# lajoiepy/cslam

Hardware: AMD Instinct MI355X
Metric: keyframes/sec (extract+match) on 100kx4096-D bank (higher is better)
Workload: dtype f32

## Files before the change

cslam_amd/_lib.py:

```python
import ctypes as C
import os
import subprocess

_HERE = os.path.dirname(os.path.abspath(__file__))
LIB_PATH = os.environ.get("CSLAM_HIP_LIB") or os.path.join(_HERE, "libcslam_hip.so")
CSRC_DIR = os.path.join(_HERE, "csrc")

F32, F64 = 0, 1
MODE_AUTO, MODE_SCAN, MODE_MFMA = 0, 1, 2


class CslamHipError(RuntimeError):
    pass


class CslamGraphError(CslamHipError):
    """CSLAM_E_GRAPH: the graph admits no Fiedler pair (not connected, singular junction Laplacian, TraceMIN breakdown) --
    the condition under which the reference's networkx call raises and acm.py:436-466 re-draws its start point.  Not a
    failure of the GPU path."""


class CslamUnsupportedError(CslamHipError):
    """CSLAM_E_UNSUPPORTED: an optional run-time dependency (RCCL, rocBLAS / rocSOLVER) was not found on this host."""


class CslamLimitError(CslamHipError):
    """CSLAM_E_LIMIT: valid input beyond a size limit of this entry point (cslam_fiedler: junctions of the dense factor)."""


_ERROR_CLASSES = {-5: CslamUnsupportedError, -6: CslamGraphError, -7: CslamLimitError}

_lib = None

_vp, _i, _i64, _f = C.c_void_p, C.c_int, C.c_int64, C.c_float
_SIGNATURES = {
    "cslam_last_error": (C.c_char_p, []),
    "cslam_version": (_i, []),
    "cslam_device_count": (_i, [C.POINTER(_i)]),
    "cslam_device_info": (_i, [_i, C.c_char_p, _i, C.POINTER(_i64), C.POINTER(_i)]),
    "cslam_bank_create": (_i, [_i, _i, _i64, C.POINTER(_vp)]),
    "cslam_bank_destroy": (_i, [_vp]),
    "cslam_bank_size": (_i, [_vp, C.POINTER(_i64), C.POINTER(_i)]),
    "cslam_bank_clear": (_i, [_vp]),
    "cslam_bank_add_host": (_i, [_vp, _vp, _i, _i64]),
    "cslam_bank_add_dev": (_i, [_vp, _vp, _i64, _i64, _vp]),
    "cslam_bank_read_host": (_i, [_vp, _i64, _i64, _vp]),
    "cslam_bank_device_ptr": (_i, [_vp, C.POINTER(_vp), C.POINTER(_i64)]),
    "cslam_bank_search_host": (_i, [_vp, _vp, _i, _i64, _i, _vp, _i, _vp, _vp, _vp]),
    "cslam_bank_search_dev": (_i, [_vp, _vp, _i, _i64, _i64, _i, _vp, _i, _vp, _vp, _vp, _vp]),
    "cslam_bank_search_multi_dev": (_i, [_vp, _i, _vp, _i, _i64, _i64, _vp, _vp, _i, _vp, _vp, _vp, _vp]),
    "cslam_bank_search_enqueue_dev": (_i, [_vp, _vp, _i, _i64, _i64, _i, _vp, _i, _vp, _vp, _vp, _vp]),
    "cslam_bank_search_finish": (_i, [_vp, C.POINTER(_i64)]),
    "cslam_bank_search_flag_copy_dev": (_i, [_vp, _vp, _vp]),
    "cslam_bank_search_multi_enqueue_dev": (_i, [_vp, _i, _vp, _i, _i64, _i64, _vp, _vp, _i, _vp, _vp, _vp, _vp]),
    "cslam_bank_search_multi_finish": (_i, [_vp, _i, C.POINTER(_i64)]),
    "cslam_bank_last_stats": (_i, [_vp, C.POINTER(_i64 * 4)]),
    "cslam_bank_last_stage": (_i, [_vp, C.POINTER(C.c_int32 * 4)]),
    "cslam_bank_last_kernel_ms": (_i, [_vp, C.POINTER(_f)]),
    "cslam_topk_merge_dev": (_i, [_vp, _vp, _vp, _vp, _i, _i64, _i, _vp, _vp, _vp, _vp]),
    "cslam_l2_normalize_dev": (_i, [_vp, _i64, _i, _i64, _f, _i, _vp]),
    "cslam_vlad_aggregate_dev": (_i, [_vp, _vp, _vp, _vp, _i, _i, _i, _i, _vp, _i64, _vp]),
    "cslam_vlad_aggregate_nhwc_dev": (_i, [_vp, _vp, _vp, _vp, _i, _i, _i, _i, _vp, _i64, _vp]),
    "cslam_gem_fc_head_dev": (_i, [_vp, _f, _f, _vp, _vp, _i, _i, _i, _i, _vp, _vp]),
    "cslam_gem_fc_head_nhwc_dev": (_i, [_vp, _f, _f, _vp, _vp, _i, _i, _i, _i, _vp, _vp]),
    "cslam_pca_project_dev": (_i, [_vp, _i64, _vp, _i64, _vp, _vp, _i, _i, _i, _vp, _vp]),
    "cslam_pca_project_pairs_dev": (_i, [_vp, _i64, C.c_float, _vp, C.c_float, _i, _vp, _vp, _i, _i, _i, _vp, _vp]),
    "cslam_preprocess_dev": (_i, [_vp, _i, _i, _i, _i, _i, C.POINTER(_f * 3), C.POINTER(_f * 3), _vp, _vp]),
    "cslam_preprocess_nhwc_dev": (_i, [_vp, _i, _i, _i, _i, _i, C.POINTER(_f * 3), C.POINTER(_f * 3), _vp, _vp]),
    "cslam_mac_grad_dev": (_i, [_vp, _vp, _vp, _vp, _i64, _vp, _vp]),
    "cslam_csr_spmm_dev": (_i, [_vp, _vp, _vp, _i64, _vp, _i, _vp, _vp]),
    "cslam_csr_spmm4_dev": (_i, [_vp, _vp, _vp, _i64, _vp, _vp, _vp]),
    "cslam_block4_gram_dev": (_i, [_vp, _vp, _i64, _vp, _vp, _vp]),
    "cslam_block4_affine_dev": (_i, [_vp, _i64, _vp, _vp, _vp, _vp]),
    "cslam_block4_residual_dev": (_i, [_vp, _vp, _i64, _vp, C.c_double, _vp, _vp, _vp]),
    "cslam_block4_gram_sync": (_i, [_vp, _vp, _i64, _vp, _vp, _vp, _vp]),
    "cslam_block4_affine_host": (_i, [_vp, _i64, _vp, _vp, _vp, _vp]),
    "cslam_block4_residual_sync": (_i, [_vp, _vp, _i64, _vp, C.c_double, _vp, _vp, _vp, _vp]),
    "cslam_chain_forward_dev": (_i, [_vp, _vp, _vp, _i64, _vp, _i, _vp, _vp, _vp, _vp, _vp, _vp, _vp, _vp, _vp, _vp, _vp]),
    "cslam_chain_backward_dev": (_i, [_vp, _vp, _vp, _vp, _vp, _vp, _vp, _vp, _vp, _vp, _i64, _vp, _vp]),
    "cslam_chol_solve4_dev": (_i, [_vp, _i64, _i64, _i, _vp, _vp, _i, _vp, _vp, _vp]),
    "cslam_fiedler": (_i, [_i64, _vp, _vp, _vp, _vp, C.c_uint32, C.c_double, _i, _vp, _vp, _vp, _vp]),
    "cslam_fiedler_start_block": (_i, [C.c_uint32, _i64, _vp]),
    "cslam_fiedler_release": (_i, []),
    "cslam_mac_fw_subset": (_i, [_i64, _i64, _vp, _vp, _vp, _i64, _vp, _vp, _vp, _vp, _i64, _i, C.c_double, C.c_double, _vp, _vp, _vp, _vp, _vp]),
    "cslam_pgo_plan": (_i, [_i64, _i64, _vp, _vp, _i64, _vp]),
    "cslam_pgo_linearize_dev": (_i, [_vp, _vp, _vp, _vp, _vp, _vp]),
    "cslam_pgo_system_host": (_i, [_vp, _vp, _vp, _vp, _vp, _vp]),
    "cslam_pgo_solve_dev": (_i, [C.c_double, _vp, _vp, _vp, _vp]),
    "cslam_pgo_retract_dev": (_i, [_vp, _vp, _i64, _vp, _vp]),
    "cslam_pgo_cost_dev": (_i, [_vp, _vp, _vp, _vp, _vp, _vp, _vp]),
    "cslam_pgo_weights_dev": (_i, [_vp, _i64, C.c_double, C.c_double, _vp, _vp, _vp]),
    "cslam_pgo_optimize": (_i, [_i64, _i64, _vp, _vp, _i64, _vp, _vp, _vp, _vp, _vp, _vp, _vp]),
    "cslam_pgo_trace": (_i, [_vp, _i64, _vp]),
    "cslam_pgo_release": (_i, []),
    "cslam_scbank_create": (_i, [_i, _i, _i, _i64, _vp]),
    "cslam_scbank_destroy": (_i, [_vp]),
    "cslam_scbank_size": (_i, [_vp, _vp, _vp, _vp]),
    "cslam_scbank_clear": (_i, [_vp]),
    "cslam_scbank_add_host": (_i, [_vp, _vp, _i64]),
    "cslam_scbank_add_dev": (_i, [_vp, _vp, _i64, _vp]),
    "cslam_scbank_read_host": (_i, [_vp, _i64, _i64, _vp, _vp]),
    "cslam_scbank_search_host": (_i, [_vp, _vp, _i64, _i, _vp, _vp, _vp, _vp, _vp, _vp, _vp]),
    "cslam_scbank_search_dev": (_i, [_vp, _vp, _i64, _i, _vp, _vp, _vp, _vp, _vp, _vp, _vp, _vp]),
    "cslam_bias_act_pool_dev": (_i, [_vp, _vp, _i, _i, _i, _i, _i, _i, _vp, _vp]),
    "cslam_conv3x3_c3_dev": (_i, [_vp, _vp, _vp, _i, _i, _i, _i, _i, _vp, _vp]),
    "cslam_wino_input_dev": (_i, [_vp, _i, _i, _i, _i, _vp, _vp]),
    "cslam_wino_output_dev": (_i, [_vp, _vp, _vp, _i, _i, _i, _i, _i, _i, _vp, _vp]),
    "cslam_wino4_input_dev": (_i, [_vp, _i, _i, _i, _i, _vp, _vp]),
    "cslam_wino4_output_dev": (_i, [_vp, _vp, _vp, _i, _i, _i, _i, _i, _i, _vp, _vp]),
    "cslam_absmax_dev": (_i, [_vp, _i64, _vp, _vp]),
    "cslam_wino4_input_h3_dev": (_i, [_vp, _i, _i, _i, _i, _vp, _vp, _vp]),
    "cslam_wino4_output_scaled_dev": (_i, [_vp, _vp, _vp, _i, _i, _i, _i, _i, _i, _vp, C.c_float, _vp, _vp, _vp]),
    "cslam_wino2_fused64_dev": (_i, [_vp, _vp, _vp, _i, _i, _i, _i, _i, _vp, _vp]),
    "cslam_wino2_fused_c64_dev": (_i, [_vp, _vp, _vp, _vp, _i, _i, _i, _i, _i, _i, _vp, _vp]),
    "cslam_wino4_fused_c64_dev": (_i, [_vp, _vp, _vp, _vp, _i, _i, _i, _i, _i, _i, _vp, _vp]),
    "cslam_scancontext_from_cloud_dev": (_i, [_vp, _vp, _i, _i, _i, C.c_double, _vp, _vp, _vp]),
    "cslam_icp_correspondences_dev": (_i, [_vp, _vp, _vp, _vp, _i, _vp, C.c_double, _vp, _vp, _vp]),
    "cslam_icp_register_dev": (_i, [_vp, _vp, _vp, _vp, _i, _vp, _vp, _vp, _i, C.c_double, C.c_double, _vp, _vp, _vp]),
    "cslam_icp_register_plane_dev": (_i, [_vp, _vp, _vp, _vp, _vp, _i, _vp, _vp, _vp, _i, C.c_double, C.c_double, _vp, _vp, _vp]),
    "cslam_voxel_downsample_dev": (_i, [_vp, _vp, _i, C.c_double, _vp, _vp, _vp, _vp, _vp, _vp]),
    "cslam_knn_radius_dev": (_i, [_vp, _vp, _i, C.c_double, _i, _vp, _vp, _vp, _vp, _vp]),
    "cslam_normals_dev": (_i, [_vp, _vp, _i, _vp, _vp, _vp, _i, C.c_double, _i, _vp, _vp, _vp, _vp]),
    "cslam_fpfh_dev": (_i, [_vp, _vp, _vp, _i, _vp, _vp, _vp, _i, _vp, _vp, _vp, _vp]),
    "cslam_feature_match_dev": (_i, [_vp, _vp, _vp, _vp, _i, _i, _vp, _vp, _vp, _vp, _vp, _vp, _vp]),
    "cslam_robust_graph_dev": (_i, [_vp, _vp, _vp, _vp, _i, C.c_double, _vp, _vp, _vp, _vp, _vp, _vp]),
    "cslam_robust_clique_dev": (_i, [_vp, _vp, _vp, _vp, _vp, _i, _i64, _vp, _vp, _vp, _vp, _vp, _vp, _vp]),
    "cslam_robust_rotation_dev": (_i, [_vp, _vp, _vp, _vp, _vp, _i, C.c_double, _vp, _vp, _vp, _vp, _vp]),
    "cslam_robust_translation_dev": (_i, [_vp, _vp, _vp, _vp, _vp, _vp, _i, C.c_double, _vp, _vp, _vp, _vp]),
    "cslam_robust_fit_dev": (_i, [_vp, _vp, _vp, _vp, _vp, _vp, _vp, _i, C.c_double, _i64, _vp, _vp, _vp, _vp, _vp, _vp]),
    "cslam_vis_match_dev": (_i, [_vp, _vp, _vp, _vp, _i, _i, C.c_double, _vp, _vp, _vp, _vp, _vp]),
    "cslam_vis_pnp_dev": (_i, [_vp, _vp, _vp, _vp, _vp, _vp, _vp, _vp, _i, _i, C.c_double, _i, _i, _i, C.c_uint64, _vp, _vp, _vp, _vp]),
    "cslam_vis_register_dev": (_i, [_vp, _vp, _vp, _vp, _vp, _vp, _vp, _i, _i, C.c_double, _i, C.c_double, _i, _i, _i, C.c_uint64,
                                    _vp, _vp, _vp, _vp, _vp, _vp, _vp, _vp]),
    "cslam_vis_hypotheses_dev": (_i, [_vp, _vp, _vp, _vp, _i, _i, C.c_double, C.c_uint64, _vp, _vp, _vp, _vp, _vp, _vp, _vp]),
    "cslam_wino4_fused_c64_h_dev": (_i, [_vp, _vp, _vp, _vp, _i, _i, _i, _i, _i, _i, _vp, C.c_float, _vp, _vp, _vp]),
    "cslam_conv3x3_direct_h_dev": (_i, [_vp, _vp, _vp, _i, _i, _i, _i, _i, _i, _i, _vp, _f, _vp, _vp, _vp]),
    "cslam_conv3x3_direct_r_dev": (_i, [_vp, _vp, _vp, _i, _i, _i, _i, _i, _i, _i, _vp, C.c_float, _vp, _vp, _vp]),
    "cslam_conv3x3_direct_r2_dev": (_i, [_vp, _vp, _vp, _i, _i, _i, _i, _i, _i, _i, _vp, C.c_float, _vp, _vp, _vp]),
    "cslam_conv_stem_direct_h_dev": (_i, [_vp, _vp, _vp, _vp, C.c_float, _vp, _vp, C.c_float, _i, _i, _i, _i, _vp, _vp, _vp, _vp]),
    "cslam_wino4_stem_c64_h_dev": (_i, [_vp, _vp, _vp, _vp, C.c_float, _vp, _vp, _i, _i, _i, _i, _vp, C.c_float, _vp, _vp, _vp]),
    "cslam_debug_wfh_prof_dev": (_i, [_vp]),
    "cslam_conv3x3_c3_amax_dev": (_i, [_vp, _vp, _vp, _i, _i, _i, _i, _i, _vp, _vp, _vp]),
    "cslam_wino4_input_h2_dev": (_i, [_vp, _i, _i, _i, _i, _vp, _vp, _vp]),
    "cslam_wino_gemm_h2_dev": (_i, [_vp, _vp, _i64, _i, _i, _vp, _vp]),
    "cslam_wino4_chain_h2_dev": (_i, [_vp, _vp, _i, _i, _i, _i, _vp, C.c_float, _vp, C.c_float, C.c_float, _vp, _vp, _vp, _vp]),
    "cslam_wino_zgemm_h2_dev": (_i, [_vp, _vp, _i64, _i, _i, _vp, _vp]),
    "cslam_wino4_output_z_dev": (_i, [_vp, _vp, _i, _i, _i, _i, _i, _i, _vp, C.c_float, _vp, _vp, _vp]),
    "cslam_conv_igemm_h2_dev": (_i, [_vp, _vp, _vp, _vp, _i, _i, _i, _i, _i, _i, _i, _i, _i, _i, _vp, C.c_float, _vp, _vp, _vp]),
    "cslam_conv_stem_pool_igemm_h2_dev": (_i, [_vp, _vp, _vp, _i, _i, _i, _i, _i, _i, _i, _i, _vp, C.c_float, _vp, _vp, _vp]),
    "cslam_conv_igemm_h2p_dev": (_i, [_vp, _i, _vp, _vp, _vp, _vp, _i, _vp, _i, _i, _i, _i, _i, _i, _i, _i, _i, _i, _vp, C.c_float,
                                      C.c_float, C.c_float, _vp, _i, _vp, _vp, _vp]),
    "cslam_conv3x3_direct_r_pairs_dev": (_i, [_vp, _vp, _vp, _i, _i, _i, _i, _i, _vp, C.c_float, C.c_float, C.c_float, _vp, _vp, _vp, _vp]),
    "cslam_conv3x3_direct_hp_dev": (_i, [_vp, _vp, _vp, _vp, _i, _i, _i, _i, _i, _i, _i, C.c_float, _vp, _vp, _vp]),
    "cslam_conv3x3_direct_p_dev": (_i, [_vp, _i, _vp, _vp, _vp, _vp, _i, _vp, _i, _i, _i, _i, _i, _i, _vp, C.c_float, C.c_float, C.c_float,
                                        _vp, _i, _vp, _vp, _vp]),
    "cslam_comm_unique_id": (_i, [_vp]),
    "cslam_comm_init": (_i, [_i, _i, _vp, _i, C.POINTER(_vp)]),
    "cslam_comm_destroy": (_i, [_vp]),
    "cslam_comm_info": (_i, [_vp, C.POINTER(_i), C.POINTER(_i)]),
    "cslam_allgather_queries_dev": (_i, [_vp, _vp, _i64, _i64, _vp, _vp]),
    "cslam_exchange_lists_dev": (_i, [_vp, _vp, _vp, _i64, _vp]),
    "cslam_peak_copy_dev": (_i, [_vp, _vp, _i64, _i, _vp]),
    "cslam_peak_mfma_dev": (_i, [_i, _i, _i, _i, _vp, C.POINTER(C.c_double), _vp]),
    "cslam_debug_last_candidates": (_i, [_vp, _i64, C.POINTER(_i), _vp, _vp, C.POINTER(C.c_double)]),
    "cslam_ring_schedule_describe": (_i, [_i, _i, _i, _i, C.POINTER(C.c_int32 * 6), _vp, _i64, _vp, _vp, _vp]),
    "cslam_trunk_timing": (_i, [_i]),
    "cslam_trunk_timing_read": (_i, [C.POINTER(C.c_double * 8)]),
    "cslam_voxel_profile": (_i, [_i]),
    "cslam_voxel_profile_read": (_i, [C.POINTER(C.c_double * 6), C.POINTER(C.c_int32 * 4)]),
}

EXPERIMENTAL_SYMBOLS = ("cslam_wino4_input_h3_dev", "cslam_wino2_fused64_dev", "cslam_wino2_fused_c64_dev",
                        "cslam_wino4_fused_c64_dev", "cslam_debug_wfh_prof_dev", "cslam_peak_copy_dev", "cslam_peak_mfma_dev",
                        "cslam_debug_last_candidates", "cslam_ring_schedule_describe", "cslam_trunk_timing", "cslam_trunk_timing_read",
                        "cslam_voxel_profile", "cslam_voxel_profile_read", "cslam_vis_hypotheses_dev")
EXPORTED_SYMBOLS = tuple(n for n in _SIGNATURES if n not in EXPERIMENTAL_SYMBOLS)


def build(verbose=False):
    r = subprocess.run(["make", "-C", CSRC_DIR, "-j", "4"], capture_output=True, text=True)
    if verbose or r.returncode != 0:
        print(r.stdout[-4000:])
        print(r.stderr[-4000:])
    if r.returncode != 0:
        raise CslamHipError("building libcslam_hip.so failed")
    return LIB_PATH


def load():
    global _lib
    if _lib is not None:
        return _lib
    try:
        import torch
    except ImportError:
        pass
    if not os.path.exists(LIB_PATH):
        raise CslamHipError(
            f"{LIB_PATH} not found: the HIP extension is not built "
            "(run `python __graft_entry__.py` or `make -C cslam_amd/csrc`); there is no CPU fallback")
    lib = C.CDLL(LIB_PATH)
    for name, (res, args) in _SIGNATURES.items():
        fn = getattr(lib, name)
        fn.restype = res
        fn.argtypes = args
    _lib = lib
    return lib


def check(rc):
    if rc != 0:
        msg = load().cslam_last_error()
        raise _ERROR_CLASSES.get(rc, CslamHipError)(f"libcslam_hip error {rc}: {msg.decode() if msg else ''}")


def require_gpu():
    lib = load()
    n = C.c_int(0)
    rc = lib.cslam_device_count(C.byref(n))
    if rc != 0 or n.value < 1:
        msg = lib.cslam_last_error()
        raise CslamHipError("no HIP device visible: cslam_amd needs an MI355X (gfx950); "
                            f"no CPU fallback exists ({msg.decode() if msg else ''})")
    return n.value
```

cslam_amd/csrc/conv_direct_r.hip:

```cpp
#include <stdlib.h>
#include <type_traits>
#include <hip/hip_fp16.h>
#include "common.h"
#include "pairs.h"

typedef float f32x4 __attribute__((ext_vector_type(4)));
typedef unsigned u32x4 __attribute__((ext_vector_type(4)));
typedef _Float16 f16x8 __attribute__((ext_vector_type(8)));
typedef float dr_f32x2 __attribute__((ext_vector_type(2)));

#define DR_PP 320
#define DR_SWZ(pc) (((pc) >> 1) & 3)
#define DR_RP (18 * DR_PP)
#define DR_PATCHB (10 * DR_RP)
#define DR_NPIX 180
#define DR_NEL 12
#define DR_SINKB 4096
#define DR_LDS (2 * DR_PATCHB + DR_SINKB)
#define DR_SINK_END (63 * 16 + 128 + 8)

struct ConvDirectRArgs {
    const float *x; const f16x8 *w2; const float *bias; float *y;
    int B, H, W, gxb, gyb, nblk;
    int relu;
    const unsigned *amax_in; float inv_sw; unsigned *amax_out;
    float wl1, bmax; unsigned *bound_out;
};

#ifdef CSLAM_ABLATIONS
__device__ unsigned long long *dr_prof = nullptr;
extern "C" __attribute__((visibility("default"))) int cslam_debug_dr_prof_dev(void *d_buf) {
    unsigned long long *q = (unsigned long long *)d_buf;
    return hipMemcpyToSymbol(HIP_SYMBOL(dr_prof), &q, sizeof(q)) == hipSuccess ? 0 : -2;
}
#define DR_PROF 1
#else
#define DR_PROF 0
#endif

template <bool POOL, bool RELU, int DBG = 0, bool OUTP = false>
__global__ __launch_bounds__(256, 1) void conv3x3_direct_r_kernel(ConvDirectRArgs p) {
    static_assert(!(POOL && OUTP), "the pair-format output is written un-pooled");
    static_assert(DR_SINK_END <= DR_SINKB, "a sink store leaves the sink");
    extern __shared__ __attribute__((aligned(16))) char dr_smem[];
    const int tid = threadIdx.x;
    const int lane = tid & 63;
    const int wave = __builtin_amdgcn_readfirstlane(tid >> 6);
    const int gq = lane >> 4, l15 = lane & 15;

    const float amax = fminf(fmaxf(__uint_as_float(*p.amax_in), 1e-30f), 1e30f);
    const float sx = scale_le_32752(__uint_as_float(*p.amax_in));
    const float inv = p.inv_sw / sx;
    float s_out = 1.0f, neg1 = -1.0f;
    asm volatile("" : "+v"(neg1));
    if (OUTP) {
        const float bound = (amax * p.wl1 + p.bmax) * 1.001f;
        s_out = scale_in_2p13_2p14(bound);
        if (blockIdx.x == 0 && threadIdx.x == 0) *p.bound_out = __float_as_uint(bound);
    }

    const bool by_xcd = (gridDim.x & 7) == 0;
    const int wg_xcd = by_xcd ? (int)blockIdx.x & 7 : 0, wg_j = by_xcd ? (int)blockIdx.x >> 3 : (int)blockIdx.x;
    const int wg_per = by_xcd ? (int)gridDim.x >> 3 : (int)gridDim.x;
    const int per_xcd = by_xcd ? (p.nblk + 7) >> 3 : p.nblk;
    const int blk_beg = wg_xcd * per_xcd;
    const int blk_cnt = min(per_xcd, p.nblk - blk_beg);
    const int n_mine = blk_cnt > wg_j ? (blk_cnt - wg_j + wg_per - 1) / wg_per : 0;
    if (n_mine <= 0) return;

    f16x8 wr[9][2][2][2];
#pragma unroll
    for (int tap = 0; tap < 9; ++tap)
#pragma unroll
        for (int ks = 0; ks < 2; ++ks)
#pragma unroll
            for (int mt = 0; mt < 2; ++mt)
#pragma unroll
                for (int hl = 0; hl < 2; ++hl) {
                    wr[tap][ks][mt][hl] = p.w2[((((wave * 9 + tap) * 2 + ks) * 2 + mt) * 2 + hl) * 64 + lane];
                    if (tap < 6) asm volatile("" : "+a"(wr[tap][ks][mt][hl]));
                }
    float4 bv[2];
#pragma unroll
    for (int mt = 0; mt < 2; ++mt)
        bv[mt] = p.bias ? *(const float4 *)(p.bias + 32 * wave + 16 * mt + 4 * gq) : make_float4(0.f, 0.f, 0.f, 0.f);

    struct Blk { int img, by, bx; };
    auto decode_blk = [&](int bi) {
        int blk = wg_j + bi * wg_per;
        blk = blk_beg + (blk < blk_cnt ? blk : blk_cnt - 1);
        const int per_img = p.gxb * p.gyb;
        Blk b;
        b.img = blk / per_img;
        const int rem = blk - b.img * per_img;
        b.by = rem / p.gxb; b.bx = rem - b.by * p.gxb;
        return b;
    };

    int st_dst[DR_NEL];
    unsigned st_pc = 0;
#pragma unroll
    for (int i = 0; i < DR_NEL; ++i) {
        const int e = i * 256 + tid, px = e >> 4, f4 = e & 15;
        const int pr = (px * 3641) >> 16, pc = px - 18 * pr;
        const bool valid = px < DR_NPIX;
        st_dst[i] = valid ? pr * DR_RP + pc * DR_PP + (((f4 >> 1) ^ DR_SWZ(pc)) << 4) + (f4 & 1) * 8 : -1;
        if (i < 6) st_pc |= (unsigned)(valid ? pc : 0) << (5 * i);
    }
    unsigned st_pc2 = 0;
#pragma unroll
    for (int i = 6; i < DR_NEL; ++i) {
        const int e = i * 256 + tid, px = e >> 4;
        const int pr = (px * 3641) >> 16, pc = px - 18 * pr;
        st_pc2 |= (unsigned)(px < DR_NPIX ? pc : 0) << (5 * (i - 6));
    }
    const int img_bytes = p.H * p.W * 256;
    u32x4 stg[DR_NEL];
    auto patch_load = [&](const Blk &b, int i) {
        const __amdgpu_buffer_rsrc_t rsX = buf_rsrc((const char *)p.x + (int64_t)b.img * img_bytes, img_bytes, RSRC_LIM16);
        const int blk_off = ((b.by * 8 - 1) * p.W + (b.bx * 16 - 1)) * 256;
        int t = tid;
        asm volatile("" : "+v"(t));
        const int e = i * 256 + t, px = e >> 4;
        const int pr = (px * 3641) >> 16, pc = px - 18 * pr;
        int off = ((pr * p.W + pc) * 64 + (e & 15) * 4) * 4 + blk_off;
        asm volatile("" : "+v"(off));
        stg[i] = __builtin_amdgcn_raw_buffer_load_b128(rsX, px < DR_NPIX ? off : 0x7fffffff, 0, 0);
    };
    auto patch_split = [&](const Blk &b, int i, char *patch) {
        const unsigned pc = __builtin_amdgcn_ubfe(i < 6 ? st_pc : st_pc2, 5 * (i < 6 ? i : i - 6), 5);
        const float s = (unsigned)(b.bx * 16 - 1) + pc < (unsigned)p.W ? sx : 0.0f;
        dr_f32x2 w01 = dr_f32x2{__uint_as_float(stg[i].x), __uint_as_float(stg[i].y)} * dr_f32x2{s, s};
        dr_f32x2 w23 = dr_f32x2{__uint_as_float(stg[i].z), __uint_as_float(stg[i].w)} * dr_f32x2{s, s};
        asm("" : "+v"(w01), "+v"(w23));
        const float w0 = w01[0], w1 = w01[1], w2 = w23[0], w3 = w23[1];
        const __half2 h01 = __floats2half2_rn(w0, w1), h23 = __floats2half2_rn(w2, w3);
        const float d0 = sub_half<0>(w0, h01), d1 = sub_half<1>(w1, h01), d2 = sub_half<0>(w2, h23), d3 = sub_half<1>(w3, h23);
        const __half2 l01 = __floats2half2_rn(d0, d1), l23 = __floats2half2_rn(d2, d3);
        char *d = st_dst[i] >= 0 ? patch + st_dst[i] : dr_smem + 2 * DR_PATCHB + (tid & 63) * 16;
        *(uint2 *)d = make_uint2(*(const unsigned *)&h01, *(const unsigned *)&h23);
        *(uint2 *)(d + 128) = make_uint2(*(const unsigned *)&l01, *(const unsigned *)&l23);
    };

    f32x4 acc[8][2];
    int fr_off[3];
#pragma unroll
    for (int dx = 0; dx < 3; ++dx) fr_off[dx] = (l15 + dx) * DR_PP + ((gq ^ DR_SWZ(l15 + dx)) << 4);
    f16x8 fh[3], fl[3];
    auto frag_read = [&](auto col_tag, auto r_tag, const char *patch) {
        constexpr int COL = decltype(col_tag)::value, R = decltype(r_tag)::value;
        constexpr int DX = COL >> 1, KS = COL & 1, SLOT = (R + COL) % 3;
        fh[SLOT] = *(const f16x8 *)(patch + fr_off[DX] + R * DR_RP + KS * 64);
        fl[SLOT] = *(const f16x8 *)(patch + fr_off[DX] + R * DR_RP + KS * 64 + 128);
    };
    float my_amax = 0.0f;
    const int Ho = POOL ? p.H >> 1 : p.H, Wo = POOL ? p.W >> 1 : p.W;
    Blk eb = {0, 0, 0};
    auto epi_rows = [&](int k) {
        const __amdgpu_buffer_rsrc_t rsY = buf_rsrc((const char *)(p.y + (int64_t)eb.img * Ho * Wo * 128), (int64_t)Ho * Wo * 512, RSRC_LIM16);
        const int ox = eb.bx * 16 + l15;
#pragma unroll
        for (int mt = 0; mt < 2; ++mt) {
            const int ch_off = (32 * wave + 16 * mt + 4 * gq) * 4;
            float4 v;
            bool store;
            int off;
            if (POOL) {
                const int py = eb.by * 4 + k;
                v.x = max_f32_xor1(max_f32(acc[2 * k][mt][0], acc[2 * k + 1][mt][0])); v.y = max_f32_xor1(max_f32(acc[2 * k][mt][1], acc[2 * k + 1][mt][1]));
                v.z = max_f32_xor1(max_f32(acc[2 * k][mt][2], acc[2 * k + 1][mt][2])); v.w = max_f32_xor1(max_f32(acc[2 * k][mt][3], acc[2 * k + 1][mt][3]));
                store = ((l15 & 1) == 0) & ((ox >> 1) < Wo) & (py < Ho);
                off = (py * Wo + (ox >> 1)) * 512 + ch_off;
            } else {
                const int oy = eb.by * 8 + k;
                v.x = acc[k][mt][0]; v.y = acc[k][mt][1]; v.z = acc[k][mt][2]; v.w = acc[k][mt][3];
                store = (ox < p.W) & (oy < p.H);
                off = (oy * p.W + ox) * 512 + ch_off;
            }
            v.x = v.x * inv + bv[mt].x; v.y = v.y * inv + bv[mt].y; v.z = v.z * inv + bv[mt].z; v.w = v.w * inv + bv[mt].w;
            if (RELU) { v.x = fmaxf(v.x, 0.0f); v.y = fmaxf(v.y, 0.0f); v.z = fmaxf(v.z, 0.0f); v.w = fmaxf(v.w, 0.0f); }
            float m = max_f32(max_f32(fabsf(v.x), fabsf(v.y)), max_f32(fabsf(v.z), fabsf(v.w)));
            asm volatile("" : "+v"(m), "+v"(off));
            my_amax = max_f32(my_amax, store ? m : 0.0f);
            if (OUTP) {
                const float u0 = v.x * s_out, u1 = v.y * s_out, u2 = v.z * s_out, u3 = v.w * s_out;
                const unsigned h01 = pack_half2(u0, u1), h23 = pack_half2(u2, u3);
                const unsigned l01 = pack_half2(fma_half<0>(h01, neg1, u0), fma_half<1>(h01, neg1, u1));
                const unsigned l23 = pack_half2(fma_half<0>(h23, neg1, u2), fma_half<1>(h23, neg1, u3));
                const int offp = store ? off - ch_off + wave * 128 + (16 * mt + 4 * gq) * 2 : 0x7fffffff;
                typedef unsigned dr_u32x2 __attribute__((ext_vector_type(2)));
                __builtin_amdgcn_raw_buffer_store_b64((dr_u32x2){h01, h23}, rsY, offp, 0, 0);
                __builtin_amdgcn_raw_buffer_store_b64((dr_u32x2){l01, l23}, rsY, offp, 64, 0);
            } else {
            u32x4 bits;
            bits.x = __float_as_uint(v.x); bits.y = __float_as_uint(v.y); bits.z = __float_as_uint(v.z); bits.w = __float_as_uint(v.w);
            if (!(DBG & 4)) __builtin_amdgcn_raw_buffer_store_b128(bits, rsY, store ? off : 0x7fffffff, 0, 0);
            else asm volatile("" :: "v"(bits));
            }
        }
    };

    auto rstep = [&](auto col_tag, auto r_tag, const char *patch, const Blk &nblk, char *npatch) {
        constexpr int COL = decltype(col_tag)::value, R = decltype(r_tag)::value;
        constexpr int DX = COL >> 1, KS = COL & 1, SLOT = (R + COL) % 3;
        if constexpr (R + 2 < 10) frag_read(col_tag, std::integral_constant<int, (R + 2) % 10>{}, patch);
        else if constexpr (COL < 5) frag_read(std::integral_constant<int, (COL + 1) % 6>{}, std::integral_constant<int, (R + 2) % 10>{}, patch);
        if constexpr (COL == 0 && R >= 1 && R <= 6 && !(DBG & 1)) { patch_load(nblk, 2 * (R - 1)); patch_load(nblk, 2 * (R - 1) + 1); }
#pragma unroll
        for (int prod = 0; prod < 3; ++prod)
#pragma unroll
            for (int dy = 0; dy < 3; ++dy)
#pragma unroll
                for (int mt = 0; mt < 2; ++mt) {
                    const int r = R - dy;
                    if (r < 0 || r > 7) continue;
                    const f16x8 a = prod == 2 ? wr[3 * dy + DX][KS][mt][1] : wr[3 * dy + DX][KS][mt][0];
                    const f16x8 b = prod == 1 ? fl[SLOT] : fh[SLOT];
                    acc[r][mt] = __builtin_amdgcn_mfma_f32_16x16x32_f16(a, b, (COL == 0 && prod == 0 && dy == 0) ? (f32x4)(0.0f) : acc[r][mt], 0, 0, 0);
                }
        if constexpr (COL >= 3 && (R == 1 || R == 3 || R == 5 || R == 7) && !(DBG & 1)) patch_split(nblk, 4 * (COL - 3) + (R - 1) / 2, npatch);
        if constexpr (COL == 5 && !POOL && R >= 3) epi_rows(R - 3);
        if constexpr (COL == 5 && POOL && (R == 4 || R == 6 || R == 8)) epi_rows((R - 4) / 2);
        __builtin_amdgcn_sched_group_barrier(0x100, 2, 0);
        __builtin_amdgcn_sched_group_barrier(0x020, 2, 0);
        constexpr int NM = 6 * ((R < 2 ? R + 1 : 3) - (R > 7 ? R - 7 : 0));
#pragma unroll
        for (int m = 0; m < NM; ++m) {
            __builtin_amdgcn_sched_group_barrier(0x008, 1, 0);
            __builtin_amdgcn_sched_group_barrier(0x002, COL == 5 ? 4 : 2, 0);
        }
        __builtin_amdgcn_sched_group_barrier(0x200, 1, 0);
        __builtin_amdgcn_sched_barrier(0);
    };
    auto column = [&](auto col_tag, const char *patch, const Blk &nblk, char *npatch) {
        rstep(col_tag, std::integral_constant<int, 0>{}, patch, nblk, npatch); rstep(col_tag, std::integral_constant<int, 1>{}, patch, nblk, npatch);
        rstep(col_tag, std::integral_constant<int, 2>{}, patch, nblk, npatch); rstep(col_tag, std::integral_constant<int, 3>{}, patch, nblk, npatch);
        rstep(col_tag, std::integral_constant<int, 4>{}, patch, nblk, npatch); rstep(col_tag, std::integral_constant<int, 5>{}, patch, nblk, npatch);
        rstep(col_tag, std::integral_constant<int, 6>{}, patch, nblk, npatch); rstep(col_tag, std::integral_constant<int, 7>{}, patch, nblk, npatch);
        rstep(col_tag, std::integral_constant<int, 8>{}, patch, nblk, npatch); rstep(col_tag, std::integral_constant<int, 9>{}, patch, nblk, npatch);
    };
#define DR_C(T) std::integral_constant<int, T>{}

    [[maybe_unused]] unsigned long long t_main = 0, t_epi = 0, t_bar = 0, t1 = 0, t2 = 0, t3 = 0;
    Blk cb = decode_blk(0);
#pragma unroll
    for (int i = 0; i < DR_NEL; ++i) patch_load(cb, i);
#pragma unroll
    for (int i = 0; i < DR_NEL; ++i) patch_split(cb, i, dr_smem);
    __syncthreads();
    for (int bi = 0; bi < n_mine; ++bi) {
        const int cur = bi & 1;
        const char *const patch = dr_smem + cur * DR_PATCHB;
        char *const npatch = dr_smem + (cur ^ 1) * DR_PATCHB;
        const Blk nb = decode_blk(bi + 1);
        eb = cb;
        if (DR_PROF) t1 = __builtin_amdgcn_s_memtime();
        frag_read(DR_C(0), DR_C(0), patch);
        frag_read(DR_C(0), DR_C(1), patch);
        column(DR_C(0), patch, nb, npatch); column(DR_C(1), patch, nb, npatch); column(DR_C(2), patch, nb, npatch);
        column(DR_C(3), patch, nb, npatch); column(DR_C(4), patch, nb, npatch); column(DR_C(5), patch, nb, npatch);
        if (DR_PROF) { t2 = __builtin_amdgcn_s_memtime(); t_main += t2 - t1; }
        epi_rows(POOL ? 3 : 7);
        if (DR_PROF) { t3 = __builtin_amdgcn_s_memtime(); t_epi += t3 - t2; }
        __syncthreads();
        if (DR_PROF) t_bar += __builtin_amdgcn_s_memtime() - t3;
        cb = nb;
    }
#ifdef CSLAM_ABLATIONS
    if (dr_prof && blockIdx.x == 0 && tid == 0) { dr_prof[0] = t_main; dr_prof[1] = t_epi; dr_prof[2] = t_bar; dr_prof[3] = (unsigned long long)n_mine; }
#endif

    if (p.amax_out) {
        unsigned *s_amax = (unsigned *)dr_smem;
        if (tid == 0) *s_amax = 0u;
        __syncthreads();
#pragma unroll
        for (int o = 32; o > 0; o >>= 1) my_amax = fmaxf(my_amax, __shfl_xor(my_amax, o, 64));
        if (lane == 0) atomicMax(s_amax, __float_as_uint(my_amax));
        __syncthreads();
        if (tid == 0 && *s_amax > *(volatile unsigned *)p.amax_out) atomicMax(p.amax_out, *s_amax);
    }
}

typedef float f32x2 __attribute__((ext_vector_type(2)));
#define DR2_SINKB 1280
#define DR2_BUF (DR_PATCHB + DR2_SINKB)
#define DR2_LDS (2 * DR2_BUF)
struct ConvDirectR2Args {
    const float *x; const f16x8 *w2; const float *bias; float *y;
    int B, H, W, gxb, gyb, nblk;
    const unsigned *amax_in; float inv_sw; unsigned *amax_out;
};
template <bool POOL, bool RELU, int DBG = 0>
__global__ __launch_bounds__(256, 1) void conv3x3_direct_r2_kernel(ConvDirectR2Args p) {
    extern __shared__ __attribute__((aligned(16))) char dr_smem[];
    const int tid = threadIdx.x;
    const int lane = tid & 63;
    const int wave = __builtin_amdgcn_readfirstlane(tid >> 6);
    const int gq = lane >> 4, l15 = lane & 15;

    const float sx = scale_le_32752(__uint_as_float(*p.amax_in));
    const float inv = p.inv_sw / sx;

    const bool by_xcd = (gridDim.x & 15) == 0;
    const int wg_xcd = by_xcd ? (int)blockIdx.x & 7 : 0, wg_raw = by_xcd ? (int)blockIdx.x >> 3 : (int)blockIdx.x;
    const int half = wg_raw & 1, wg_j = wg_raw >> 1;
    const int wg_per = (by_xcd ? (int)gridDim.x >> 3 : (int)gridDim.x) >> 1;
    const int per_xcd = by_xcd ? (p.nblk + 7) >> 3 : p.nblk;
    const int blk_beg = wg_xcd * per_xcd;
    const int blk_cnt = min(per_xcd, p.nblk - blk_beg);
    const int n_mine = blk_cnt > wg_j ? (blk_cnt - wg_j + wg_per - 1) / wg_per : 0;
    if (n_mine <= 0) return;

    f16x8 wr[9][2][2][2];
#pragma unroll
    for (int tap = 0; tap < 9; ++tap)
#pragma unroll
        for (int ks = 0; ks < 2; ++ks)
#pragma unroll
            for (int sl = 0; sl < 2; ++sl)
#pragma unroll
                for (int hl = 0; hl < 2; ++hl) {
                    wr[tap][ks][sl][hl] = p.w2[((((((half * 4 + wave) * 9 + tap) * 2 + ks) * 2 + sl) * 2 + hl) * 64) + lane];
                    if (tap < 7) asm volatile("" : "+a"(wr[tap][ks][sl][hl]));
                }
    const float4 bv = p.bias ? *(const float4 *)(p.bias + 64 * half + 16 * wave + 4 * gq) : make_float4(0.f, 0.f, 0.f, 0.f);

    struct Blk { int img, by, bx; };
    auto decode_blk = [&](int bi) {
        int blk = wg_j + bi * wg_per;
        blk = blk_beg + (blk < blk_cnt ? blk : blk_cnt - 1);
        const int per_img = p.gxb * p.gyb;
        Blk b;
        b.img = blk / per_img;
        const int rem = blk - b.img * per_img;
        b.by = rem / p.gxb; b.bx = rem - b.by * p.gxb;
        return b;
    };

    static_assert(DR_SINK_END <= DR2_SINKB && DR2_BUF % 256 == 0, "a sink store leaves its sink, or the second buffer moves in the banks");
    int st_dst[DR_NEL], st_src[DR_NEL];
    unsigned st_pc = 0, st_pc2 = 0;
#pragma unroll
    for (int i = 0; i < DR_NEL; ++i) {
        const int e = i * 256 + tid, px = e >> 4, f4 = e & 15;
        const int pr = (px * 3641) >> 16, pc = px - 18 * pr;
        const bool valid = px < DR_NPIX;
        st_dst[i] = valid ? pr * DR_RP + pc * DR_PP + (((f4 >> 1) ^ DR_SWZ(pc)) << 4) + (f4 & 1) * 8 : DR_PATCHB + (tid & 63) * 16;
        st_src[i] = valid ? ((pr * p.W + pc) * 128 + f4 * 4) * 4 : -1;
        if (i < 6) st_pc |= (unsigned)(valid ? pc : 0) << (5 * i);
        else st_pc2 |= (unsigned)(valid ? pc : 0) << (5 * (i - 6));
    }
    const int img_bytes = p.H * p.W * 512;
    u32x4 stg[DR_NEL];
    auto patch_load = [&](const Blk &b, int slab, int i) {
        const __amdgpu_buffer_rsrc_t rsX = buf_rsrc((const char *)p.x + (int64_t)b.img * img_bytes, img_bytes, RSRC_LIM16);
        const int blk_off = ((b.by * 8 - 1) * p.W + (b.bx * 16 - 1)) * 512 + slab * 256;
        int off = st_src[i] + blk_off;
        asm volatile("" : "+v"(off));
        stg[i] = __builtin_amdgcn_raw_buffer_load_b128(rsX, st_src[i] >= 0 ? off : 0x7fffffff, 0, 0);
    };
    auto patch_split = [&](const Blk &b, int i, char *patch) {
        const unsigned pc = __builtin_amdgcn_ubfe(i < 6 ? st_pc : st_pc2, 5 * (i < 6 ? i : i - 6), 5);
        const float s = (unsigned)(b.bx * 16 - 1) + pc < (unsigned)p.W ? sx : 0.0f;
        f32x2 w01 = f32x2{__uint_as_float(stg[i].x), __uint_as_float(stg[i].y)} * f32x2{s, s};
        f32x2 w23 = f32x2{__uint_as_float(stg[i].z), __uint_as_float(stg[i].w)} * f32x2{s, s};
        asm("" : "+v"(w01), "+v"(w23));
        const __half2 h01 = __floats2half2_rn(w01[0], w01[1]), h23 = __floats2half2_rn(w23[0], w23[1]);
        const float d0 = sub_half<0>(w01[0], h01), d1 = sub_half<1>(w01[1], h01), d2 = sub_half<0>(w23[0], h23), d3 = sub_half<1>(w23[1], h23);
        const __half2 l01 = __floats2half2_rn(d0, d1), l23 = __floats2half2_rn(d2, d3);
        char *d = patch + st_dst[i];
        *(uint2 *)d = make_uint2(*(const unsigned *)&h01, *(const unsigned *)&h23);
        *(uint2 *)(d + 128) = make_uint2(*(const unsigned *)&l01, *(const unsigned *)&l23);
    };

    f32x4 acc[8];
    int fr_off[3];
#pragma unroll
    for (int dx = 0; dx < 3; ++dx) fr_off[dx] = (l15 + dx) * DR_PP + ((gq ^ DR_SWZ(l15 + dx)) << 4);
    f16x8 fh[3], fl[3];
    auto frag_read = [&](auto col_tag, auto r_tag, const char *patch) {
        constexpr int COL = decltype(col_tag)::value, R = decltype(r_tag)::value;
        constexpr int DX = COL >> 1, KS = COL & 1, SLOT = (R + COL) % 3;
        fh[SLOT] = *(const f16x8 *)(patch + fr_off[DX] + R * DR_RP + KS * 64);
        fl[SLOT] = *(const f16x8 *)(patch + fr_off[DX] + R * DR_RP + KS * 64 + 128);
    };
    float my_amax = 0.0f;
    const int Ho = POOL ? p.H >> 1 : p.H, Wo = POOL ? p.W >> 1 : p.W;
    Blk eb = {0, 0, 0};
    auto epi_rows = [&](int k) {
        const __amdgpu_buffer_rsrc_t rsY = buf_rsrc((const char *)(p.y + (int64_t)eb.img * Ho * Wo * 128), (int64_t)Ho * Wo * 512, RSRC_LIM16);
        const int ox = eb.bx * 16 + l15;
        const int ch_off = (64 * half + 16 * wave + 4 * gq) * 4;
        float4 v;
        bool store;
        int off;
        if (POOL) {
            const int py = eb.by * 4 + k;
            v.x = max_f32_xor1(max_f32(acc[2 * k][0], acc[2 * k + 1][0])); v.y = max_f32_xor1(max_f32(acc[2 * k][1], acc[2 * k + 1][1]));
            v.z = max_f32_xor1(max_f32(acc[2 * k][2], acc[2 * k + 1][2])); v.w = max_f32_xor1(max_f32(acc[2 * k][3], acc[2 * k + 1][3]));
            store = ((l15 & 1) == 0) & ((ox >> 1) < Wo) & (py < Ho);
            off = (py * Wo + (ox >> 1)) * 512 + ch_off;
        } else {
            const int oy = eb.by * 8 + k;
            v.x = acc[k][0]; v.y = acc[k][1]; v.z = acc[k][2]; v.w = acc[k][3];
            store = (ox < p.W) & (oy < p.H);
            off = (oy * p.W + ox) * 512 + ch_off;
        }
        v.x = v.x * inv + bv.x; v.y = v.y * inv + bv.y; v.z = v.z * inv + bv.z; v.w = v.w * inv + bv.w;
        if (RELU) { v.x = fmaxf(v.x, 0.0f); v.y = fmaxf(v.y, 0.0f); v.z = fmaxf(v.z, 0.0f); v.w = fmaxf(v.w, 0.0f); }
        float m = max_f32(max_f32(fabsf(v.x), fabsf(v.y)), max_f32(fabsf(v.z), fabsf(v.w)));
        asm volatile("" : "+v"(m), "+v"(off));
        my_amax = max_f32(my_amax, store ? m : 0.0f);
        u32x4 bits;
        bits.x = __float_as_uint(v.x); bits.y = __float_as_uint(v.y); bits.z = __float_as_uint(v.z); bits.w = __float_as_uint(v.w);
        if (!(DBG & 4)) __builtin_amdgcn_raw_buffer_store_b128(bits, rsY, store ? off : 0x7fffffff, 0, 0);
        else asm volatile("" :: "v"(bits));
    };

    auto rstep = [&](auto col_tag, auto r_tag, auto slab_tag, const char *patch, const Blk &nblk, int nslab, char *npatch) {
        constexpr int COL = decltype(col_tag)::value, R = decltype(r_tag)::value, SL = decltype(slab_tag)::value;
        constexpr int DX = COL >> 1, KS = COL & 1, SLOT = (R + COL) % 3;
        if constexpr (R + 2 < 10) frag_read(col_tag, std::integral_constant<int, (R + 2) % 10>{}, patch);
        else if constexpr (COL < 5) frag_read(std::integral_constant<int, (COL + 1) % 6>{}, std::integral_constant<int, (R + 2) % 10>{}, patch);
        if constexpr (COL == 0 && R >= 1 && R <= 6 && !(DBG & 1) && !(DBG & 8)) { patch_load(nblk, nslab, 2 * (R - 1)); patch_load(nblk, nslab, 2 * (R - 1) + 1); }
#pragma unroll
        for (int prod = 0; prod < 3; ++prod)
#pragma unroll
            for (int dy = 0; dy < 3; ++dy) {
                const int r = R - dy;
                if (r < 0 || r > 7) continue;
                const f16x8 a = prod == 2 ? wr[3 * dy + DX][KS][SL][1] : wr[3 * dy + DX][KS][SL][0];
                const f16x8 b = prod == 1 ? fl[SLOT] : fh[SLOT];
                acc[r] = __builtin_amdgcn_mfma_f32_16x16x32_f16(a, b, (SL == 0 && COL == 0 && prod == 0 && dy == 0) ? (f32x4)(0.0f) : acc[r], 0, 0, 0);
            }
        if constexpr (COL >= 3 && (R == 1 || R == 3 || R == 5 || R == 7) && !(DBG & 1) && !(DBG & 16)) patch_split(nblk, 4 * (COL - 3) + (R - 1) / 2, npatch);
        if constexpr (SL == 1 && COL == 5 && !POOL && R >= 3) epi_rows(R - 3);
        if constexpr (SL == 1 && COL == 5 && POOL && (R == 4 || R == 6 || R == 8)) epi_rows((R - 4) / 2);
        __builtin_amdgcn_sched_group_barrier(0x100, 2, 0);
        __builtin_amdgcn_sched_group_barrier(0x020, 2, 0);
        constexpr int NM = 3 * ((R < 2 ? R + 1 : 3) - (R > 7 ? R - 7 : 0));
#pragma unroll
        for (int m = 0; m < NM; ++m) {
            __builtin_amdgcn_sched_group_barrier(0x008, 1, 0);
            __builtin_amdgcn_sched_group_barrier(0x002, (SL == 1 && COL == 5) ? 8 : 4, 0);
        }
        __builtin_amdgcn_sched_group_barrier(0x200, 1, 0);
        __builtin_amdgcn_sched_barrier(0);
    };
    auto column = [&](auto col_tag, auto slab_tag, const char *patch, const Blk &nblk, int nslab, char *npatch) {
        rstep(col_tag, std::integral_constant<int, 0>{}, slab_tag, patch, nblk, nslab, npatch); rstep(col_tag, std::integral_constant<int, 1>{}, slab_tag, patch, nblk, nslab, npatch);
        rstep(col_tag, std::integral_constant<int, 2>{}, slab_tag, patch, nblk, nslab, npatch); rstep(col_tag, std::integral_constant<int, 3>{}, slab_tag, patch, nblk, nslab, npatch);
        rstep(col_tag, std::integral_constant<int, 4>{}, slab_tag, patch, nblk, nslab, npatch); rstep(col_tag, std::integral_constant<int, 5>{}, slab_tag, patch, nblk, nslab, npatch);
        rstep(col_tag, std::integral_constant<int, 6>{}, slab_tag, patch, nblk, nslab, npatch); rstep(col_tag, std::integral_constant<int, 7>{}, slab_tag, patch, nblk, nslab, npatch);
        rstep(col_tag, std::integral_constant<int, 8>{}, slab_tag, patch, nblk, nslab, npatch); rstep(col_tag, std::integral_constant<int, 9>{}, slab_tag, patch, nblk, nslab, npatch);
    };
    auto pass = [&](auto slab_tag, const char *patch, const Blk &nblk, int nslab, char *npatch) {
        frag_read(DR_C(0), DR_C(0), patch);
        frag_read(DR_C(0), DR_C(1), patch);
        column(DR_C(0), slab_tag, patch, nblk, nslab, npatch); column(DR_C(1), slab_tag, patch, nblk, nslab, npatch);
        column(DR_C(2), slab_tag, patch, nblk, nslab, npatch); column(DR_C(3), slab_tag, patch, nblk, nslab, npatch);
        column(DR_C(4), slab_tag, patch, nblk, nslab, npatch); column(DR_C(5), slab_tag, patch, nblk, nslab, npatch);
    };

    Blk cb = decode_blk(0);
#pragma unroll
    for (int i = 0; i < DR_NEL; ++i) patch_load(cb, 0, i);
#pragma unroll
    for (int i = 0; i < DR_NEL; ++i) patch_split(cb, i, dr_smem);
    __syncthreads();
    char *const buf0 = dr_smem, *const buf1 = dr_smem + DR2_BUF;
    for (int bi = 0; bi < n_mine; ++bi) {
        const Blk nb = decode_blk(bi + 1);
        eb = cb;
        pass(DR_C(0), buf0, cb, 1, buf1);
        __syncthreads();
        pass(DR_C(1), buf1, nb, 0, buf0);
        epi_rows(POOL ? 3 : 7);
        __syncthreads();
        cb = nb;
    }
    if (p.amax_out) {
        unsigned *s_amax = (unsigned *)dr_smem;
        if (tid == 0) *s_amax = 0u;
        __syncthreads();
#pragma unroll
        for (int o = 32; o > 0; o >>= 1) my_amax = fmaxf(my_amax, __shfl_xor(my_amax, o, 64));
        if (lane == 0) atomicMax(s_amax, __float_as_uint(my_amax));
        __syncthreads();
        if (tid == 0 && *s_amax > *(volatile unsigned *)p.amax_out) atomicMax(p.amax_out, *s_amax);
    }
}

CSLAM_API int cslam_conv3x3_direct_r2_dev(const float *d_x, const void *d_w2r2, const float *d_bias, int B, int H, int W, int Cin,
                                          int Cout, int relu, int pool, const unsigned *d_amax, float inv_sw,
                                          unsigned *d_amax_out, float *d_y, void *stream) {
    PTR_DEVICE(d_x);
    ARG_CHECK(d_x && d_w2r2 && d_y && d_amax, "NULL argument");
    ARG_CHECK(B >= 1 && H >= 1 && W >= 1, "empty map");
    ARG_CHECK(Cin == 128 && Cout == 128, "Cin and Cout must be 128");
    ARG_CHECK(!pool || ((H % 2) == 0 && (W % 2) == 0), "pooling needs even H and W");
    ARG_CHECK(inv_sw > 0.0f, "inv_sw must be positive");
    ARG_CHECK((int64_t)H * W * 512 < 0x7ffffff0ll, "one image's maps must stay below 2 GiB (32-bit buffer offsets)");
    ConvDirectR2Args a;
    a.x = d_x; a.w2 = (const f16x8 *)d_w2r2; a.bias = d_bias; a.y = d_y;
    a.B = B; a.H = H; a.W = W;
    a.gxb = (int)ceil_div64(W, 16); a.gyb = (int)ceil_div64(H, 8);
    const int64_t nblk = (int64_t)B * a.gxb * a.gyb;
    ARG_CHECK(nblk < (1ll << 30), "too many blocks for one launch");
    a.nblk = (int)nblk;
    a.amax_in = d_amax; a.inv_sw = inv_sw; a.amax_out = d_amax_out;
    const int n_cu = cslam_cu_count();
    ARG_CHECK(n_cu >= 2, "no HIP device");
    int grid = n_cu % 16 == 0 ? n_cu : (n_cu & ~1);
    if (2 * nblk < grid) grid = (int)(2 * nblk);
    hipStream_t st = (hipStream_t)stream;
#define DR2_LAUNCH(P, R) do { \
        static DeviceOnce once; int once_dev; \
        if (once.todo(&once_dev)) { \
            HIP_TRY(hipFuncSetAttribute((const void *)conv3x3_direct_r2_kernel<P, R>, hipFuncAttributeMaxDynamicSharedMemorySize, DR2_LDS)); \
            once.done(once_dev); } \
        hipLaunchKernelGGL((conv3x3_direct_r2_kernel<P, R>), dim3(grid), dim3(256), DR2_LDS, st, a); } while (0)
#ifdef CSLAM_ABLATIONS
    if (const char *e = getenv("CSLAM_DR_DBG")) {
        const int d = atoi(e);
#define DR2_LAUNCH_D(D) do { HIP_TRY(hipFuncSetAttribute((const void *)conv3x3_direct_r2_kernel<true, true, D>, hipFuncAttributeMaxDynamicSharedMemorySize, DR2_LDS)); \
        hipLaunchKernelGGL((conv3x3_direct_r2_kernel<true, true, D>), dim3(grid), dim3(256), DR2_LDS, st, a); HIP_TRY(hipGetLastError()); return CSLAM_OK; } while (0)
        if (d == 1) DR2_LAUNCH_D(1);
        if (d == 4) DR2_LAUNCH_D(4);
        if (d == 5) DR2_LAUNCH_D(5);
        if (d == 8) DR2_LAUNCH_D(8);
        if (d == 16) DR2_LAUNCH_D(16);
#undef DR2_LAUNCH_D
    }
#endif
    if (pool && relu) DR2_LAUNCH(true, true);
    else if (pool) DR2_LAUNCH(true, false);
    else if (relu) DR2_LAUNCH(false, true);
    else DR2_LAUNCH(false, false);
#undef DR2_LAUNCH
    HIP_TRY(hipGetLastError());
    return CSLAM_OK;
}

static int conv_direct_r_launch(const float *d_x, const void *d_w2r, const float *d_bias, int B, int H, int W, int Cin,
                                int Cout, int relu, int pool, const unsigned *d_amax, float inv_sw,
                                unsigned *d_amax_out, float *d_y, void *stream, int out_pairs, float wl1, float bmax, unsigned *d_bound_out) {
    PTR_DEVICE(d_x);
    ARG_CHECK(!out_pairs || (!pool && relu && d_bound_out && wl1 >= 0.0f && bmax >= 0.0f), "pair-format output: ReLU, no pooling, wl1, bmax and the bound slot");
    ARG_CHECK(d_x && d_w2r && d_y && d_amax, "NULL argument");
    ARG_CHECK(B >= 1 && H >= 1 && W >= 1, "empty map");
    ARG_CHECK(Cin == 64 && Cout == 128, "Cin must be 64 and Cout 128");
    ARG_CHECK(!pool || ((H % 2) == 0 && (W % 2) == 0), "pooling needs even H and W");
    ARG_CHECK(inv_sw > 0.0f, "inv_sw must be positive");
    ARG_CHECK((int64_t)H * W * 512 < 0x7ffffff0ll, "one image's maps must stay below 2 GiB (32-bit buffer offsets)");
    ConvDirectRArgs a;
    a.x = d_x; a.w2 = (const f16x8 *)d_w2r; a.bias = d_bias; a.y = d_y;
    a.B = B; a.H = H; a.W = W;
    a.gxb = (int)ceil_div64(W, 16); a.gyb = (int)ceil_div64(H, 8);
    const int64_t nblk = (int64_t)B * a.gxb * a.gyb;
    ARG_CHECK(nblk < (1ll << 30), "too many blocks for one launch");
    a.nblk = (int)nblk;
    a.relu = relu; a.amax_in = d_amax; a.inv_sw = inv_sw; a.amax_out = d_amax_out;
    a.wl1 = wl1; a.bmax = bmax; a.bound_out = d_bound_out;
    const int n_cu = cslam_cu_count();
    ARG_CHECK(n_cu > 0, "no HIP device");
    const int grid = (int)(nblk < n_cu ? nblk : n_cu);
    hipStream_t st = (hipStream_t)stream;
    if (out_pairs) {
        static DeviceOnce once_p; int once_dev_p;
        if (once_p.todo(&once_dev_p)) {
            HIP_TRY(hipFuncSetAttribute((const void *)conv3x3_direct_r_kernel<false, true, 0, true>, hipFuncAttributeMaxDynamicSharedMemorySize, DR_LDS));
            once_p.done(once_dev_p); }
        hipLaunchKernelGGL((conv3x3_direct_r_kernel<false, true, 0, true>), dim3(grid), dim3(256), DR_LDS, st, a);
        HIP_TRY(hipGetLastError());
        return CSLAM_OK;
    }
#define DR_LAUNCH(P, R) do { \
        static DeviceOnce once; int once_dev; \
        if (once.todo(&once_dev)) { \
            HIP_TRY(hipFuncSetAttribute((const void *)conv3x3_direct_r_kernel<P, R>, hipFuncAttributeMaxDynamicSharedMemorySize, DR_LDS)); \
            once.done(once_dev); } \
        hipLaunchKernelGGL((conv3x3_direct_r_kernel<P, R>), dim3(grid), dim3(256), DR_LDS, st, a); } while (0)
#ifdef CSLAM_ABLATIONS
    if (const char *e = getenv("CSLAM_DR_DBG")) {
        const int d = atoi(e);
#define DR_LAUNCH_D(D) do { HIP_TRY(hipFuncSetAttribute((const void *)conv3x3_direct_r_kernel<false, true, D>, hipFuncAttributeMaxDynamicSharedMemorySize, DR_LDS)); \
        hipLaunchKernelGGL((conv3x3_direct_r_kernel<false, true, D>), dim3(grid), dim3(256), DR_LDS, st, a); HIP_TRY(hipGetLastError()); return CSLAM_OK; } while (0)
        if (d == 1) DR_LAUNCH_D(1);
        if (d == 4) DR_LAUNCH_D(4);
        if (d == 5) DR_LAUNCH_D(5);
#undef DR_LAUNCH_D
    }
#endif
    if (pool && relu) DR_LAUNCH(true, true);
    else if (pool) DR_LAUNCH(true, false);
    else if (relu) DR_LAUNCH(false, true);
    else DR_LAUNCH(false, false);
#undef DR_LAUNCH
    HIP_TRY(hipGetLastError());
    return CSLAM_OK;
}
CSLAM_API int cslam_conv3x3_direct_r_dev(const float *d_x, const void *d_w2r, const float *d_bias, int B, int H, int W, int Cin,
                                         int Cout, int relu, int pool, const unsigned *d_amax, float inv_sw,
                                         unsigned *d_amax_out, float *d_y, void *stream) {
    return conv_direct_r_launch(d_x, d_w2r, d_bias, B, H, W, Cin, Cout, relu, pool, d_amax, inv_sw, d_amax_out, d_y, stream, 0, 0.0f, 0.0f, nullptr);
}
CSLAM_API int cslam_conv3x3_direct_r_pairs_dev(const float *d_x, const void *d_w2r, const float *d_bias, int B, int H, int W, int Cin,
                                               int Cout, const unsigned *d_amax, float inv_sw, float wl1, float bmax,
                                               unsigned *d_amax_out, unsigned *d_bound_out, void *d_y, void *stream) {
    return conv_direct_r_launch(d_x, d_w2r, d_bias, B, H, W, Cin, Cout, 1, 0, d_amax, inv_sw, d_amax_out, (float *)d_y, stream, 1, wl1, bmax, d_bound_out);
}
```

cslam_amd/csrc/conv_stem_direct_h.hip:

```cpp
#include <stdlib.h>
#include <type_traits>
#include <hip/hip_fp16.h>
#include "common.h"
#include "pairs.h"

typedef float f32x4 __attribute__((ext_vector_type(4)));
typedef unsigned u32x4 __attribute__((ext_vector_type(4)));
typedef _Float16 f16x8 __attribute__((ext_vector_type(8)));

#define SD_PP 320
#define SD_SWZ(pc) (((pc) >> 1) & 3)
#define SD_RP (18 * SD_PP)
#define SD_PATCHB (10 * SD_RP)
#define SD_IW 20
#define SD_IMG (12 * SD_IW * 3)
#define SD_T9 (20 * 17)
#define SD_IMGB (SD_IMG + SD_T9)
#define SD_NPIX 180
#define SD_LDS (2 * SD_PATCHB + 2 * SD_IMGB * 4)

struct StemDirectArgs {
    const float *x0; const unsigned *w1; const float *b1; const float *sumw; float inv_sw1;
    const f16x8 *w2; const float *bias; float inv_sw2;
    int B, H, W, gxb, gyb, nblk;
    const unsigned *amax_in; unsigned *amax_out; float *y;
};

#ifdef CSLAM_ABLATIONS
__device__ unsigned long long *sd_prof = nullptr;
extern "C" __attribute__((visibility("default"))) int cslam_debug_sd_prof_dev(void *d_buf) {
    unsigned long long *q = (unsigned long long *)d_buf;
    return hipMemcpyToSymbol(HIP_SYMBOL(sd_prof), &q, sizeof(q)) == hipSuccess ? 0 : -2;
}
#define SD_PROF 1
#else
#define SD_PROF 0
#endif

template <bool POOL, int DBG = 0>
__global__ __launch_bounds__(256, 1) void conv_stem_direct_h_kernel(StemDirectArgs p) {
    extern __shared__ __attribute__((aligned(16))) char sd_smem[];
    const int tid = threadIdx.x;
    const int lane = tid & 63;
    const int wave = __builtin_amdgcn_readfirstlane(tid >> 6);
    const int gq = lane >> 4, l15 = lane & 15;
    unsigned *const s_img_all = (unsigned *)(sd_smem + 2 * SD_PATCHB);

    const float a0 = fminf(fmaxf(__uint_as_float(*p.amax_in), 1e-30f), 1e30f);
    int e_;
    (void)frexpf(16384.0f / a0, &e_);
    const float s1 = ldexpf(1.0f, e_ - 1);
    const float inv1 = p.inv_sw1 / s1;
    float bound = 0.0f;
    for (int c = 0; c < 64; ++c) bound = fmaxf(bound, fabsf(p.b1 ? p.b1[c] : 0.0f) + a0 * p.sumw[c]);
    bound = fminf(fmaxf(bound, 1e-30f), 1e30f);
    (void)frexpf(32752.0f / bound, &e_);
    const float sx = ldexpf(1.0f, e_ - 1);
    const float inv2 = p.inv_sw2 / sx;

    const bool by_xcd = (gridDim.x & 7) == 0;
    const int wg_xcd = by_xcd ? (int)blockIdx.x & 7 : 0, wg_j = by_xcd ? (int)blockIdx.x >> 3 : (int)blockIdx.x;
    const int wg_per = by_xcd ? (int)gridDim.x >> 3 : (int)gridDim.x;
    const int per_xcd = by_xcd ? (p.nblk + 7) >> 3 : p.nblk;
    const int blk_beg = wg_xcd * per_xcd;
    const int blk_cnt = min(per_xcd, p.nblk - blk_beg);
    const int n_mine = blk_cnt > wg_j ? (blk_cnt - wg_j + wg_per - 1) / wg_per : 0;
    if (n_mine <= 0) return;

    f16x8 wr[9][2][2];
#pragma unroll
    for (int tap = 0; tap < 9; ++tap)
#pragma unroll
        for (int ks = 0; ks < 2; ++ks)
#pragma unroll
            for (int hl = 0; hl < 2; ++hl) {
                wr[tap][ks][hl] = p.w2[(((wave * 9 + tap) * 2 + ks) * 2 + hl) * 64 + lane];
                asm volatile("" : "+a"(wr[tap][ks][hl]));
            }
    const u32x4 w1h = ((const u32x4 *)p.w1)[(wave * 2 + 0) * 64 + lane], w1l = ((const u32x4 *)p.w1)[(wave * 2 + 1) * 64 + lane];
    const f16x8 W1h = __builtin_bit_cast(f16x8, w1h), W1l = __builtin_bit_cast(f16x8, w1l);
    const float k1 = inv1 * sx;
    float b1s[4];
#pragma unroll
    for (int r = 0; r < 4; ++r) b1s[r] = (p.b1 ? p.b1[16 * wave + 4 * gq + r] : 0.0f) * sx;
    float4 bv2;
    bv2 = p.bias ? *(const float4 *)(p.bias + 16 * wave + 4 * gq) : make_float4(0.f, 0.f, 0.f, 0.f);

    int e_dst[3], e_rc[3];
#pragma unroll
    for (int j = 0; j < 3; ++j) {
        const int e = j * 256 + tid;
        const int ci = (e >= 240) + (e >= 480);
        const int rem = e - 240 * ci;
        const int r = (rem * 3277) >> 16, c = rem - 20 * r;
        e_dst[j] = e < SD_IMG ? (r * SD_IW + c) * 3 + ci : -1;
        e_rc[j] = (ci << 16) | (r << 8) | c;
    }
    struct Blk { int img, by, bx; };
    auto decode_blk = [&](int bi) {
        int blk = wg_j + bi * wg_per;
        blk = blk_beg + (blk < blk_cnt ? blk : blk_cnt - 1);
        const int per_img = p.gxb * p.gyb;
        Blk b;
        b.img = blk / per_img;
        const int rem = blk - b.img * per_img;
        b.by = rem / p.gxb; b.bx = rem - b.by * p.gxb;
        return b;
    };
    float raw[3];
    auto img_load = [&](const Blk &b) {
#pragma unroll
        for (int j = 0; j < 3; ++j) {
            const int ci = e_rc[j] >> 16, r = (e_rc[j] >> 8) & 255, c = e_rc[j] & 255;
            const int gy = b.by * 8 - 2 + r, gx = b.bx * 16 - 2 + c;
            const bool in = (e_dst[j] >= 0) & (gy >= 0) & (gy < p.H) & (gx >= 0) & (gx < p.W);
            raw[j] = in ? p.x0[((int64_t)(b.img * 3 + ci) * p.H + gy) * p.W + gx] : 0.0f;
        }
    };
    auto img_store = [&](unsigned *s_img) {
#pragma unroll
        for (int j = 0; j < 3; ++j)
            if (e_dst[j] >= 0) {
                const unsigned v = pack_pair(raw[j] * s1);
                s_img[e_dst[j]] = v;
                if ((e_rc[j] >> 16) == 2) s_img[SD_IMG + (e_rc[j] & 255) * 17 + ((e_rc[j] >> 8) & 255)] = v;
            }
    };

    int c1_src[12], c1_dst[12];
#pragma unroll
    for (int t = 0; t < 12; ++t) {
        int pp = 16 * t + l15;
        pp = pp < SD_NPIX ? pp : SD_NPIX - 1;
        const int pr = (pp * 3641) >> 16, pc = pp - 18 * pr;
        c1_src[t] = (gq < 3 ? ((pr + gq) * SD_IW + pc) * 3 : SD_IMG + (pc + 2) * 17 + pr) * 4;
        c1_dst[t] = pr * SD_RP + pc * SD_PP + (((2 * wave + (gq >> 1)) ^ SD_SWZ(pc)) << 4) + (gq & 1) * 8;
    }
    for (int i = tid; i < 2 * 20 * 5; i += 256)
        s_img_all[(i / 100) * SD_IMGB + SD_IMG + ((i % 100) / 5) * 17 + 12 + (i % 5)] = 0u;
    unsigned pk[2][8];
    auto conv1_read = [&](int g, const unsigned *s_img) {
#pragma unroll
        for (int i = 0; i < 2; ++i) {
            const unsigned *ib = (const unsigned *)((const char *)s_img + c1_src[2 * g + i]);
#pragma unroll
            for (int j = 0; j < 8; ++j) pk[i][j] = ib[j];
        }
    };
    f32x4 c1[2];
    float c1v[2][4];
    auto conv1_piece = [&](int g, int piece, const Blk &b, char *patch) {
        const int i = piece & 1;
        if (piece < 2) {
            u32x4 ah, al;
#pragma unroll
            for (int d = 0; d < 4; ++d) {
                ah[d] = __builtin_amdgcn_perm(pk[i][2 * d + 1], pk[i][2 * d], 0x05040100u);
                al[d] = __builtin_amdgcn_perm(pk[i][2 * d + 1], pk[i][2 * d], 0x07060302u);
            }
            const f16x8 Ph = __builtin_bit_cast(f16x8, ah), Pl = __builtin_bit_cast(f16x8, al);
            c1[i] = __builtin_amdgcn_mfma_f32_16x16x32_f16(W1l, Ph, (f32x4)(0.0f), 0, 0, 0);
            c1[i] = __builtin_amdgcn_mfma_f32_16x16x32_f16(W1h, Pl, c1[i], 0, 0, 0);
            c1[i] = __builtin_amdgcn_mfma_f32_16x16x32_f16(W1h, Ph, c1[i], 0, 0, 0);
            asm volatile("" : "+v"(c1[i]));
            return;
        }
        if (piece < 4) {
#pragma unroll
            for (int r = 0; r < 4; ++r) c1v[i][r] = fmaxf(c1[i][r] * k1 + b1s[r], 0.0f);
            return;
        }
        const __half2 h01 = __floats2half2_rn(c1v[i][0], c1v[i][1]), h23 = __floats2half2_rn(c1v[i][2], c1v[i][3]);
        const float d0 = sub_half<0>(c1v[i][0], h01), d1 = sub_half<1>(c1v[i][1], h01);
        const float d2 = sub_half<0>(c1v[i][2], h23), d3 = sub_half<1>(c1v[i][3], h23);
        const __half2 l01 = __floats2half2_rn(d0, d1), l23 = __floats2half2_rn(d2, d3);
        if ((DBG & 16) == 0 && (2 * g + i < 11 || l15 < 4)) {
            char *d = patch + c1_dst[2 * g + i];
            *(uint2 *)d = make_uint2(*(const unsigned *)&h01, *(const unsigned *)&h23);
            *(uint2 *)(d + 128) = make_uint2(*(const unsigned *)&l01, *(const unsigned *)&l23);
        }
    };
    auto border_fixup = [&](const Blk &b, char *patch) {
        const int gy0 = b.by * 8 - 1, gx0 = b.bx * 16 - 1;
        if ((gy0 >= 0) & (gy0 + 10 <= p.H) & (gx0 >= 0) & (gx0 + 18 <= p.W)) return;
#pragma unroll
        for (int k = 0; k < 3; ++k) {
            const int pp = lane + 64 * k;
            const int pr = (pp * 3641) >> 16, pc = pp - 18 * pr;
            const int gy = gy0 + pr, gx = gx0 + pc;
            if (pp < SD_NPIX && !((gy >= 0) & (gy < p.H) & (gx >= 0) & (gx < p.W))) {
                char *d = patch + pr * SD_RP + pc * SD_PP;
                const int c0 = ((2 * wave) ^ SD_SWZ(pc)) << 4, c1_ = ((2 * wave + 1) ^ SD_SWZ(pc)) << 4;
                *(uint4 *)(d + c0) = make_uint4(0u, 0u, 0u, 0u); *(uint4 *)(d + c1_) = make_uint4(0u, 0u, 0u, 0u);
                *(uint4 *)(d + 128 + c0) = make_uint4(0u, 0u, 0u, 0u); *(uint4 *)(d + 128 + c1_) = make_uint4(0u, 0u, 0u, 0u);
            }
        }
    };

    float my_amax = 0.0f;
    const int Ho = POOL ? p.H >> 1 : p.H, Wo = POOL ? p.W >> 1 : p.W;
    f32x4 eacc[8];
    Blk ecb = {0, 0, 0};
    bool e_ok = false;
    auto epi_piece = [&](int k) {
        const __amdgpu_buffer_rsrc_t rsY = buf_rsrc((const char *)(p.y + (int64_t)ecb.img * Ho * Wo * 64), (int64_t)Ho * Wo * 256, RSRC_LIM16);
        const int ox = ecb.bx * 16 + l15;
        const int ch_off = (16 * wave + 4 * gq) * 4;
        if (POOL) {
            const int py = ecb.by * 4 + k;
            float4 v;
            v.x = max_f32_xor1(max_f32(eacc[2 * k][0], eacc[2 * k + 1][0])); v.y = max_f32_xor1(max_f32(eacc[2 * k][1], eacc[2 * k + 1][1]));
            v.z = max_f32_xor1(max_f32(eacc[2 * k][2], eacc[2 * k + 1][2])); v.w = max_f32_xor1(max_f32(eacc[2 * k][3], eacc[2 * k + 1][3]));
            v.x = fmaxf(v.x * inv2 + bv2.x, 0.0f); v.y = fmaxf(v.y * inv2 + bv2.y, 0.0f);
            v.z = fmaxf(v.z * inv2 + bv2.z, 0.0f); v.w = fmaxf(v.w * inv2 + bv2.w, 0.0f);
            const bool store = e_ok & ((l15 & 1) == 0) & ((ox >> 1) < Wo) & (py < Ho);
            float m = max_f32(max_f32(v.x, v.y), max_f32(v.z, v.w));
            int off = (py * Wo + (ox >> 1)) * 256 + ch_off;
            asm volatile("" : "+v"(m), "+v"(off));
            my_amax = max_f32(my_amax, store ? m : 0.0f);
            u32x4 bits;
            bits.x = __float_as_uint(v.x); bits.y = __float_as_uint(v.y); bits.z = __float_as_uint(v.z); bits.w = __float_as_uint(v.w);
            if (!(DBG & 4)) __builtin_amdgcn_raw_buffer_store_b128(bits, rsY, store ? off : 0x7fffffff, 0, 0);
        } else {
#pragma unroll
            for (int r = 2 * k; r < 2 * k + 2; ++r) {
                const int oy = ecb.by * 8 + r;
                float4 v;
                v.x = fmaxf(eacc[r][0] * inv2 + bv2.x, 0.0f); v.y = fmaxf(eacc[r][1] * inv2 + bv2.y, 0.0f);
                v.z = fmaxf(eacc[r][2] * inv2 + bv2.z, 0.0f); v.w = fmaxf(eacc[r][3] * inv2 + bv2.w, 0.0f);
                const bool store = e_ok & (ox < p.W) & (oy < p.H);
                float m = max_f32(max_f32(v.x, v.y), max_f32(v.z, v.w));
                int off = (oy * p.W + ox) * 256 + ch_off;
                asm volatile("" : "+v"(m), "+v"(off));
                my_amax = max_f32(my_amax, store ? m : 0.0f);
                u32x4 bits;
                bits.x = __float_as_uint(v.x); bits.y = __float_as_uint(v.y); bits.z = __float_as_uint(v.z); bits.w = __float_as_uint(v.w);
                __builtin_amdgcn_raw_buffer_store_b128(bits, rsY, store ? off : 0x7fffffff, 0, 0);
            }
        }
    };

    f32x4 acc[8];
    int fr_off[3];
#pragma unroll
    for (int dx = 0; dx < 3; ++dx) fr_off[dx] = (l15 + dx) * SD_PP + ((gq ^ SD_SWZ(l15 + dx)) << 4);
    f16x8 fh[3], fl[3];
    auto frag_read = [&](auto col_tag, auto r_tag, const char *patch) {
        constexpr int COL = decltype(col_tag)::value, R = decltype(r_tag)::value;
        constexpr int DX = COL >> 1, KS = COL & 1, SLOT = (R + COL) % 3;
        fh[SLOT] = *(const f16x8 *)(patch + fr_off[DX] + R * SD_RP + KS * 64);
        fl[SLOT] = *(const f16x8 *)(patch + fr_off[DX] + R * SD_RP + KS * 64 + 128);
    };
    auto rstep = [&](auto col_tag, auto r_tag, const char *patch, const unsigned *s_img, const Blk &nblk, char *npatch) {
        constexpr int COL = decltype(col_tag)::value, R = decltype(r_tag)::value;
        constexpr int DX = COL >> 1, KS = COL & 1, SLOT = (R + COL) % 3;
        if constexpr (DBG & 2) { }
        else if constexpr (R + 2 < 10) frag_read(col_tag, std::integral_constant<int, (R + 2) % 10>{}, patch);
        else if constexpr (COL < 5) frag_read(std::integral_constant<int, (COL + 1) % 6>{}, std::integral_constant<int, (R + 2) % 10>{}, patch);
        if constexpr (R == 0 && !(DBG & 1) && !(DBG & 8)) conv1_read(COL, s_img);
#pragma unroll
        for (int prod = 0; prod < 3; ++prod)
#pragma unroll
            for (int dy = 0; dy < 3; ++dy) {
                const int r = R - dy;
                if (r < 0 || r > 7) continue;
                const f16x8 a = prod == 2 ? wr[3 * dy + DX][KS][1] : wr[3 * dy + DX][KS][0];
                const f16x8 b = prod == 1 ? fl[SLOT] : fh[SLOT];
                acc[r] = __builtin_amdgcn_mfma_f32_16x16x32_f16(a, b, (COL == 0 && prod == 0 && dy == 0) ? (f32x4)(0.0f) : acc[r], 0, 0, 0);
            }
        if constexpr (R >= 2 && R <= 7 && !(DBG & 1)) conv1_piece(COL, R - 2, nblk, npatch);
        if constexpr (COL < 2 && (R == 1 || R == 8)) epi_piece(2 * COL + (R == 8 ? 1 : 0));
        __builtin_amdgcn_sched_group_barrier(0x100, R == 0 ? 18 : 2, 0);
        constexpr int NM = 3 * ((R < 2 ? R + 1 : 3) - (R > 7 ? R - 7 : 0)) + ((R == 2 || R == 3) ? 3 : 0);
#pragma unroll
        for (int m = 0; m < NM; ++m) {
            __builtin_amdgcn_sched_group_barrier(0x008, 1, 0);
            __builtin_amdgcn_sched_group_barrier(0x002, (COL < 2 && (R == 1 || R == 8)) ? 6 : 3, 0);
        }
        __builtin_amdgcn_sched_group_barrier(0x200, 2, 0);
        __builtin_amdgcn_sched_barrier(0);
    };
    auto edge = [&](auto col_tag, const char *patch, const unsigned *s_img) {
        constexpr int COL = decltype(col_tag)::value;
        constexpr int DX = COL >> 1, KS = COL & 1, SLOT = (9 + COL) % 3;
        constexpr int DX2 = (COL + 1) >> 1, KS2 = (COL + 1) & 1, SLOT2 = (COL + 1) % 3;
        if constexpr (!(DBG & 2)) frag_read(std::integral_constant<int, COL + 1>{}, std::integral_constant<int, 1>{}, patch);
        if constexpr (!(DBG & 1) && !(DBG & 8)) conv1_read(COL + 1, s_img);
#pragma unroll
        for (int prod = 0; prod < 3; ++prod) {
            acc[7] = __builtin_amdgcn_mfma_f32_16x16x32_f16(prod == 2 ? wr[6 + DX][KS][1] : wr[6 + DX][KS][0], prod == 1 ? fl[SLOT] : fh[SLOT], acc[7], 0, 0, 0);
            acc[0] = __builtin_amdgcn_mfma_f32_16x16x32_f16(prod == 2 ? wr[DX2][KS2][1] : wr[DX2][KS2][0], prod == 1 ? fl[SLOT2] : fh[SLOT2], acc[0], 0, 0, 0);
        }
        if constexpr (!(DBG & 2)) frag_read(std::integral_constant<int, COL + 1>{}, std::integral_constant<int, 2>{}, patch);
        __builtin_amdgcn_sched_group_barrier(0x100, 10, 0);
#pragma unroll
        for (int m = 0; m < 6; ++m) {
            __builtin_amdgcn_sched_group_barrier(0x008, 1, 0);
            __builtin_amdgcn_sched_group_barrier(0x002, 3, 0);
        }
        __builtin_amdgcn_sched_barrier(0);
    };
    auto column = [&](auto col_tag, const char *patch, const unsigned *s_img, const Blk &nblk, char *npatch) {
        constexpr int COL_ = decltype(col_tag)::value;
        if constexpr (COL_ == 0) rstep(col_tag, std::integral_constant<int, 0>{}, patch, s_img, nblk, npatch);
        rstep(col_tag, std::integral_constant<int, 1>{}, patch, s_img, nblk, npatch);
        rstep(col_tag, std::integral_constant<int, 2>{}, patch, s_img, nblk, npatch); rstep(col_tag, std::integral_constant<int, 3>{}, patch, s_img, nblk, npatch);
        rstep(col_tag, std::integral_constant<int, 4>{}, patch, s_img, nblk, npatch); rstep(col_tag, std::integral_constant<int, 5>{}, patch, s_img, nblk, npatch);
        rstep(col_tag, std::integral_constant<int, 6>{}, patch, s_img, nblk, npatch); rstep(col_tag, std::integral_constant<int, 7>{}, patch, s_img, nblk, npatch);
        rstep(col_tag, std::integral_constant<int, 8>{}, patch, s_img, nblk, npatch);
        if constexpr (COL_ == 5) rstep(col_tag, std::integral_constant<int, 9>{}, patch, s_img, nblk, npatch);
        else edge(col_tag, patch, s_img);
    };
#define SD_C(T) std::integral_constant<int, T>{}

    [[maybe_unused]] unsigned long long t_main = 0, t_epi = 0, t_bar = 0, t1 = 0, t2 = 0, t3 = 0;
    Blk cb = decode_blk(0);
    img_load(cb);
    img_store(s_img_all);
    Blk nb = decode_blk(1);
    img_load(nb);
    __syncthreads();
#pragma unroll
    for (int g = 0; g < 6; ++g) {
        conv1_read(g, s_img_all);
#pragma unroll
        for (int piece = 0; piece < 6; ++piece) conv1_piece(g, piece, cb, sd_smem);
        __builtin_amdgcn_sched_barrier(0);
    }
    border_fixup(cb, sd_smem);
    img_store(s_img_all + SD_IMGB);
    __syncthreads();
    for (int bi = 0; bi < n_mine; ++bi) {
        const int cur = bi & 1;
        const char *const patch = sd_smem + cur * SD_PATCHB;
        char *const npatch = sd_smem + (cur ^ 1) * SD_PATCHB;
        const unsigned *const s_img_next = s_img_all + (cur ^ 1) * SD_IMGB;
        const Blk nnb = decode_blk(bi + 2);
        img_load(nnb);
        if (SD_PROF) t1 = __builtin_amdgcn_s_memtime();
        frag_read(SD_C(0), SD_C(0), patch);
        frag_read(SD_C(0), SD_C(1), patch);
        column(SD_C(0), patch, s_img_next, nb, npatch); column(SD_C(1), patch, s_img_next, nb, npatch); column(SD_C(2), patch, s_img_next, nb, npatch);
        column(SD_C(3), patch, s_img_next, nb, npatch); column(SD_C(4), patch, s_img_next, nb, npatch); column(SD_C(5), patch, s_img_next, nb, npatch);
        if (!(DBG & 1)) border_fixup(nb, npatch);
        if (SD_PROF) { t2 = __builtin_amdgcn_s_memtime(); t_main += t2 - t1; }
        img_store(s_img_all + cur * SD_IMGB);
#pragma unroll
        for (int r = 0; r < 8; ++r) eacc[r] = acc[r];
        ecb = cb;
        e_ok = true;
        if (SD_PROF) { t3 = __builtin_amdgcn_s_memtime(); t_epi += t3 - t2; }
        __syncthreads();
        if (SD_PROF) t_bar += __builtin_amdgcn_s_memtime() - t3;
        cb = nb;
        nb = nnb;
    }
#pragma unroll
    for (int k = 0; k < 4; ++k) epi_piece(k);
#ifdef CSLAM_ABLATIONS
    if (sd_prof && blockIdx.x == 0 && tid == 0) { sd_prof[0] = t_main; sd_prof[1] = t_epi; sd_prof[2] = t_bar; sd_prof[3] = 0; sd_prof[4] = (unsigned long long)n_mine; }
#endif

    if (p.amax_out) {
        __syncthreads();
        unsigned *s_amax = (unsigned *)sd_smem;
        if (tid == 0) *s_amax = 0u;
        __syncthreads();
#pragma unroll
        for (int o = 32; o > 0; o >>= 1) my_amax = fmaxf(my_amax, __shfl_xor(my_amax, o, 64));
        if (lane == 0) atomicMax(s_amax, __float_as_uint(my_amax));
        __syncthreads();
        if (tid == 0 && *s_amax > *(volatile unsigned *)p.amax_out) atomicMax(p.amax_out, *s_amax);
    }
}

CSLAM_API int cslam_conv_stem_direct_h_dev(const float *d_x0, const void *d_w1, const float *d_b1, const float *d_sumw, float inv_sw1,
                                           const void *d_w2r, const float *d_bias, float inv_sw2, int B, int H, int W, int pool,
                                           const unsigned *d_amax_x0, unsigned *d_amax_out, float *d_y, void *stream) {
    PTR_DEVICE(d_x0);
    ARG_CHECK(d_x0 && d_w1 && d_sumw && d_w2r && d_y && d_amax_x0, "NULL argument");
    ARG_CHECK(B >= 1 && H >= 1 && W >= 1, "empty map");
    ARG_CHECK(!pool || ((H % 2) == 0 && (W % 2) == 0), "pooling needs even H and W");
    ARG_CHECK(inv_sw1 > 0.0f && inv_sw2 > 0.0f, "scales must be positive");
    ARG_CHECK((int64_t)H * W * 256 < 0x7ffffff0ll, "one image's output map must stay below 2 GiB (32-bit buffer offsets)");
    StemDirectArgs a;
    a.x0 = d_x0; a.w1 = (const unsigned *)d_w1; a.b1 = d_b1; a.sumw = d_sumw; a.inv_sw1 = inv_sw1;
    a.w2 = (const f16x8 *)d_w2r; a.bias = d_bias; a.inv_sw2 = inv_sw2;
    a.B = B; a.H = H; a.W = W;
    a.gxb = (int)ceil_div64(W, 16); a.gyb = (int)ceil_div64(H, 8);
    const int64_t nblk = (int64_t)B * a.gxb * a.gyb;
    ARG_CHECK(nblk < (1ll << 30), "too many blocks for one launch");
    a.nblk = (int)nblk;
    a.amax_in = d_amax_x0; a.amax_out = d_amax_out; a.y = d_y;
    const int n_cu = cslam_cu_count();
    ARG_CHECK(n_cu > 0, "no HIP device");
    const int grid = (int)(nblk < n_cu ? nblk : n_cu);
    hipStream_t st = (hipStream_t)stream;
    constexpr int lds = SD_LDS;
#define SD_LAUNCH(P) do { \
        static DeviceOnce once; int once_dev; \
        if (once.todo(&once_dev)) { \
            HIP_TRY(hipFuncSetAttribute((const void *)conv_stem_direct_h_kernel<P>, hipFuncAttributeMaxDynamicSharedMemorySize, lds)); \
            once.done(once_dev); } \
        hipLaunchKernelGGL((conv_stem_direct_h_kernel<P>), dim3(grid), dim3(256), lds, st, a); } while (0)
#ifdef CSLAM_ABLATIONS
    if (const char *e = getenv("CSLAM_SD_DBG")) {
        const int d = atoi(e);
#define SD_LAUNCH_D(D) do { HIP_TRY(hipFuncSetAttribute((const void *)conv_stem_direct_h_kernel<true, D>, hipFuncAttributeMaxDynamicSharedMemorySize, lds)); \
        hipLaunchKernelGGL((conv_stem_direct_h_kernel<true, D>), dim3(grid), dim3(256), lds, st, a); HIP_TRY(hipGetLastError()); return CSLAM_OK; } while (0)
        if (d == 1) SD_LAUNCH_D(1);
        if (d == 2) SD_LAUNCH_D(2);
        if (d == 3) SD_LAUNCH_D(3);
        if (d == 4) SD_LAUNCH_D(4);
        if (d == 7) SD_LAUNCH_D(7);
        if (d == 8) SD_LAUNCH_D(8);
        if (d == 16) SD_LAUNCH_D(16);
        if (d == 24) SD_LAUNCH_D(24);
#undef SD_LAUNCH_D
    }
#endif
    if (pool) SD_LAUNCH(true);
    else SD_LAUNCH(false);
#undef SD_LAUNCH
    HIP_TRY(hipGetLastError());
    return CSLAM_OK;
}
```

cslam_amd/vpr/conv_kernels.py:

```python
import torch

from .. import _lib
from .heads import _p, _stream


def _po(t):
    return _p(t) if t is not None else None


def _out(B, C, H, W, pool, device):
    Ho, Wo = (H // 2, W // 2) if pool else (H, W)
    return torch.empty((B, C, Ho, Wo), dtype=torch.float32, device=device, memory_format=torch.channels_last)


def _amax_slot(x, slot, have=False):
    if not have and x.numel() % 4 == 0:
        _lib.check(_lib.load().cslam_absmax_dev(_p(x), x.numel(), _p(slot), _stream(x)))
    elif not have:
        slot.copy_(x.abs().max().reshape(1))
    return slot


def stem_pool_fits(Ho, Wo):
    return Ho % 8 == 0 and Wo % 16 == 0


def conv_igemm(ws, x, Wg, bias, kernel, stride, pad, relu, residual=None, amax_in=None, amax_out=None, pool=False):
    lib = _lib.load()
    x = x.contiguous(memory_format=torch.channels_last)
    B, Cin, H, W = x.shape
    W2, inv_sw = Wg
    Cout = W2.shape[0]
    KH, KW = kernel
    Ho, Wo = (H + 2 * pad - KH) // stride + 1, (W + 2 * pad - KW) // stride + 1
    s = _stream(x)
    slot = amax_in if amax_in is not None else _amax_slot(x, ws._buf("amax", 1, x.device))
    if pool:
        assert Cin == 3 and relu and residual is None and stem_pool_fits(Ho, Wo)
        y = _out(B, Cout, Ho, Wo, True, x.device)
        _lib.check(lib.cslam_conv_stem_pool_igemm_h2_dev(_p(x), _p(W2), _po(bias), B, H, W, Cout, KH, KW, stride, pad, _p(slot),
                                                         float(inv_sw), _po(amax_out), _p(y), s))
        return y
    y = _out(B, Cout, Ho, Wo, False, x.device)
    residual = _residual_like(residual, y)
    _lib.check(lib.cslam_conv_igemm_h2_dev(_p(x), _p(W2), _po(bias), _po(residual), B, H, W, Cin, Cout, KH, KW, stride, pad,
                                           int(relu), _p(slot), float(inv_sw), _po(amax_out), _p(y), s))
    return y


class PairAct(object):
    __slots__ = ("t", "pairs", "shape", "amax", "bound")

    def __init__(self, t, pairs, shape, amax, bound):
        self.t, self.pairs, self.shape, self.amax, self.bound = t, pairs, tuple(shape), amax, bound


def pairs_to_float(act):
    B, C, H, W = act.shape
    e = torch.frexp(act.bound.view(torch.float32).clamp(1e-30, 1e30))[1].item()
    s = 2.0 ** (14 - e)
    v = (act.t[:, :, :, :, 0, :].float() + act.t[:, :, :, :, 1, :].float()) / s
    return v.reshape(B, H, W, C).permute(0, 3, 1, 2)


def _pair_out(B, Cout, Ho, Wo, out_pairs, device):
    if out_pairs:
        return torch.empty((B, Ho, Wo, Cout // 32, 2, 32), dtype=torch.float16, device=device)
    return _out(B, Cout, Ho, Wo, False, device)


def _res_args(res, shape):
    if res is None:
        return None, 0, None
    assert res.shape == shape and (res.pairs or res.t.is_contiguous(memory_format=torch.channels_last))
    return _p(res.t), int(res.pairs), _p(res.bound)


def conv_igemm_p(ws, act, Wg, bias, kernel, stride, pad, relu, res, wl1, bmax, amax_out, bound_out, out_pairs):
    B, Cin, H, W = act.shape
    W2, inv_sw = Wg
    Cout = W2.shape[0]
    KH, KW = kernel
    Ho, Wo = (H + 2 * pad - KH) // stride + 1, (W + 2 * pad - KW) // stride + 1
    y = _pair_out(B, Cout, Ho, Wo, out_pairs, act.t.device)
    rt, rpairs, rbound = _res_args(res, (B, Cout, Ho, Wo))
    assert act.pairs or act.t.is_contiguous(memory_format=torch.channels_last)
    _lib.check(_lib.load().cslam_conv_igemm_h2p_dev(
        _p(act.t), int(act.pairs), _p(act.bound), _p(W2), _po(bias), rt, rpairs, rbound, B, H, W, Cin, Cout, KH, KW, stride, pad,
        int(relu), _p(act.amax), float(inv_sw), float(wl1), float(bmax), _p(amax_out), int(out_pairs),
        _p(bound_out) if out_pairs else None, _p(y), _stream(act.t)))
    return PairAct(y, bool(out_pairs), (B, Cout, Ho, Wo), amax_out, bound_out if out_pairs else amax_out)


def conv3x3_direct_p(act, Wp, bias, relu, res, wl1, bmax, amax_out, bound_out, out_pairs):
    B, Cin, H, W = act.shape
    assert Cin == 64 and (act.pairs or (res is None and act.t.is_contiguous(memory_format=torch.channels_last)))
    y = _pair_out(B, 64, H, W, out_pairs, act.t.device)
    rt, rpairs, rbound = _res_args(res, (B, 64, H, W))
    _lib.check(_lib.load().cslam_conv3x3_direct_p_dev(
        _p(act.t), int(act.pairs), _p(act.bound), _p(Wp[0]), _po(bias), rt, rpairs, rbound, B, H, W, 64, 64, int(relu),
        _p(act.amax), float(Wp[1]), float(wl1), float(bmax), _p(amax_out), int(out_pairs), _p(bound_out) if out_pairs else None,
        _p(y), _stream(act.t)))
    return PairAct(y, bool(out_pairs), (B, 64, H, W), amax_out, bound_out if out_pairs else amax_out)


def direct_p_fits(conv_shape, kernel, stride, pad, H, W):
    return (tuple(conv_shape[:2]) == (64, 64) and tuple(kernel) == (3, 3) and stride == 1 and pad == 1
            and H * W * 512 + 11 * W * 256 < 2 ** 31 - 16)


def conv3x3_direct_h(x, Wd, bias, relu, pool, amax_in, amax_out=None):
    x = x.contiguous(memory_format=torch.channels_last)
    B, Cin, H, W = x.shape
    W2, inv_sw = Wd
    Cout = W2.shape[1]
    y = _out(B, Cout, H, W, pool, x.device)
    _lib.check(_lib.load().cslam_conv3x3_direct_h_dev(_p(x), _p(W2), _po(bias), B, H, W, Cin, Cout, int(relu), int(pool), _p(amax_in),
                                                      float(inv_sw), _po(amax_out), _p(y), _stream(x)))
    return y


def _direct_r(fn, x, Wr, bias, relu, pool, amax_in, amax_out):
    x = x.contiguous(memory_format=torch.channels_last)
    B, Cin, H, W = x.shape
    y = _out(B, 128, H, W, pool, x.device)
    _lib.check(fn(_p(x), _p(Wr[0]), _po(bias), B, H, W, Cin, 128, int(relu), int(pool), _p(amax_in), float(Wr[1]), _po(amax_out),
                  _p(y), _stream(x)))
    return y


def conv3x3_direct_r(x, Wr, bias, relu, pool, amax_in, amax_out=None):
    return _direct_r(_lib.load().cslam_conv3x3_direct_r_dev, x, Wr, bias, relu, pool, amax_in, amax_out)


def conv3x3_direct_r2(x, Wr2, bias, relu, pool, amax_in, amax_out=None):
    return _direct_r(_lib.load().cslam_conv3x3_direct_r2_dev, x, Wr2, bias, relu, pool, amax_in, amax_out)


def conv3x3_direct_r_pairs(x, Wr, bias, wl1, bmax, amax_in, bound_out, amax_out=None):
    x = x.contiguous(memory_format=torch.channels_last)
    B, Cin, H, W = x.shape
    y = torch.empty((B, H, W, 4, 2, 32), dtype=torch.float16, device=x.device)
    _lib.check(_lib.load().cslam_conv3x3_direct_r_pairs_dev(_p(x), _p(Wr[0]), _po(bias), B, H, W, Cin, 128, _p(amax_in), float(Wr[1]),
                                                            float(wl1), float(bmax), _po(amax_out), _p(bound_out), _p(y), _stream(x)))
    return y


def conv3x3_direct_hp(xp, shape, bound, Wd, bias, relu, pool, amax_out=None):
    B, Cin, H, W = shape
    W2, inv_sw = Wd
    Cout = W2.shape[1]
    y = _out(B, Cout, H, W, pool, xp.device)
    _lib.check(_lib.load().cslam_conv3x3_direct_hp_dev(_p(xp), _p(bound), _p(W2), _po(bias), B, H, W, Cin, Cout, int(relu), int(pool),
                                                       float(inv_sw), _po(amax_out), _p(y), _stream(xp)))
    return y


def conv_stem_direct_h(x0, stem, bias1, Wr, bias, pool, amax_x0, amax_out=None):
    B, C3, H, W = x0.shape
    assert C3 == 3 and x0.is_contiguous()
    y = _out(B, 64, H, W, pool, x0.device)
    _lib.check(_lib.load().cslam_conv_stem_direct_h_dev(
        _p(x0), _p(stem[0]), _po(bias1), _p(stem[2]), float(stem[1]), _p(Wr[0]), _po(bias), float(Wr[1]), B, H, W, int(pool),
        _p(amax_x0), _po(amax_out), _p(y), _stream(x0)))
    return y


def wino_stem64_h(x0, stem, bias1, Uh, bias, pool, amax_x0, amax_out=None):
    B, C3, H, W = x0.shape
    assert C3 == 3 and x0.is_contiguous() and Uh[0].shape[2] == 4
    y = _out(B, 64, H, W, pool, x0.device)
    _lib.check(_lib.load().cslam_wino4_stem_c64_h_dev(
        _p(x0), _p(stem[0]), _po(bias1), _p(stem[2]), float(stem[1]), _p(Uh[0]), _po(bias), B, H, W, int(pool), _p(amax_x0),
        float(Uh[1]), _po(amax_out), _p(y), _stream(x0)))
    return y


def _residual_like(residual, y):
    if residual is not None:
        residual = residual.contiguous(memory_format=torch.channels_last)
        assert residual.shape == y.shape
    return residual


def wino_fused64_h(x, Uh, bias, relu, pool, amax_in, amax_out=None, residual=None):
    B, _, H, W = x.shape
    Cout = Uh[0].shape[2] * 16
    y = _out(B, Cout, H, W, pool, x.device)
    residual = _residual_like(residual, y)
    _lib.check(_lib.load().cslam_wino4_fused_c64_h_dev(
        _p(x), _p(Uh[0]), _po(bias), _po(residual), B, H, W, Cout, int(relu), int(pool), _p(amax_in), float(Uh[1]), _po(amax_out),
        _p(y), _stream(x)))
    return y


def wino_fused64(x, Up, bias, relu, pool, residual=None):
    lib = _lib.load()
    B, _, H, W = x.shape
    Cout = Up.shape[2] * 16
    y = _out(B, Cout, H, W, pool, x.device)
    residual = _residual_like(residual, y)
    fn = lib.cslam_wino4_fused_c64_dev if Up.shape[1] == 36 else lib.cslam_wino2_fused_c64_dev
    _lib.check(fn(_p(x), _p(Up), _po(bias), _po(residual), B, H, W, Cout, int(relu), int(pool), _p(y), _stream(x)))
    return y
```

cslam_amd/vpr/winograd.py:

```python
import os

import torch
from torch import nn

from .. import _lib
from .conv_kernels import (PairAct, _amax_slot, _out, _po, _residual_like, conv3x3_direct_h, conv3x3_direct_hp,
                           conv3x3_direct_p, conv3x3_direct_r, conv3x3_direct_r2, conv3x3_direct_r_pairs, conv_igemm, conv_igemm_p,
                           conv_stem_direct_h, direct_p_fits, pairs_to_float, stem_pool_fits, wino_fused64, wino_fused64_h,
                           wino_stem64_h)
from .heads import _p, _stream
from .pair_weights import (direct_pair_weights, direct_r2_pair_weights, direct_r_pair_weights, fused64_pair_weights,
                           fused64_weights, igemm_pair_weights, out_bound, split16_pair_weights, split16_weights,
                           stem_direct_pair_weights, stem_pair_weights, wino_weights)


def _pair(v):
    return tuple(v) if isinstance(v, (tuple, list)) else (v, v)


_TUNED = {"done": False}


def use_tuned_gemms():
    if _TUNED["done"] or os.environ.get("CSLAM_TUNED_GEMM", "1") == "0" or not torch.cuda.is_available():
        return
    _TUNED["done"] = True
    path = os.path.join(os.path.dirname(os.path.abspath(__file__)), "tunableop_gfx950.csv")
    try:
        import torch.cuda.tunable as tunable
        if tunable.is_enabled() or not os.path.exists(path):
            return
        tunable.enable(True)
        tunable.tuning_enable(False)
        tunable.read_file(path)
    except Exception as e:
        import warnings
        warnings.warn("cslam_amd: tuned GEMM table not loaded (%s)" % e)


def _z_form(cin, cout):
    return cin * cout <= Z_FORM_MAX


Z_FORM_MAX = 128 * 128
PAIR_ACTS = True
VGG_PAIRS = False
DIRECT_P = True
IGEMM_CONVS = True


def _f4_fits(B, H, W):
    t4h, t4w = -(-H // 4), -(-W // 4)
    return B * t4h * t4w >= 512 and 16 * t4h * t4w <= 1.35 * H * W


def _pair_pipeline(ws, x, layers, slots, relu, pool, residual, amax_out):
    lib = _lib.load()
    B, Cin, H, W = x.shape
    T = B * -(-H // 4) * -(-W // 4)
    s = _stream(x)
    V2 = ws._buf("V", 36 * T * Cin, x.device)
    _lib.check(lib.cslam_wino4_input_h2_dev(_p(x), B, H, W, Cin, _p(slots[0:1]), _p(V2), s))
    vscale = slots[0:1]
    for j, (U2, bias, wl1, bmax) in enumerate(layers):
        Cout = U2[0].shape[1]
        M = ws._buf("M", 36 * T * Cout, x.device)
        _lib.check(lib.cslam_wino_gemm_h2_dev(_p(V2), _p(U2[0]), T, Cin, Cout, _p(M), s))
        if j + 1 < len(layers):
            bound = ws._buf("chain_bounds", len(layers), x.device)[j + 1:j + 2]
            V2 = ws._buf("V", 36 * T * Cout, x.device)
            _lib.check(lib.cslam_wino4_chain_h2_dev(_p(M), _po(bias), B, H, W, Cout, _p(vscale), float(U2[1]), _p(slots[j:j + 1]),
                                                    wl1, bmax, _p(slots[j + 1:j + 2]), _p(bound), _p(V2), s))
            vscale, Cin = bound, Cout
    y = _out(B, Cout, H, W, pool, x.device)
    _lib.check(lib.cslam_wino4_output_scaled_dev(_p(M), _po(bias), _po(_residual_like(residual, y)), B, H, W, Cout, int(relu),
                                                 int(pool), _p(vscale), float(U2[1]), _po(amax_out), _p(y), s))
    return y


def wino_conv3x3(ws, x, U, U4, bias, relu, pool=False, residual=None, U3=None, amax_in=None, amax_out=None, U2=None):
    lib = _lib.load()
    B, Cin, H, W = x.shape
    Cout = U.shape[2]
    assert residual is None or not pool
    four = U4 is not None and _f4_fits(B, H, W)
    ws.amax_written = four and amax_out is not None
    T = B * -(-H // 4) * -(-W // 4) if four else B * -(-H // 2) * -(-W // 2)
    s = _stream(x)
    slot = None
    if four and (U2 is not None or U3 is not None):
        slot = amax_in if amax_in is not None else _amax_slot(x, ws._buf("amax", 1, x.device))
    z = four and U2 is not None and residual is None and _z_form(Cin, Cout)
    if four and U2 is not None and not z:
        return _pair_pipeline(ws, x, [(U2, bias, None, None)], slot, relu, pool, residual, amax_out)
    inv_su = 1.0
    if z:
        V2 = ws._buf("V", 36 * T * Cin, x.device)
        M = ws._buf("M", 36 * T * Cout, x.device)
        _lib.check(lib.cslam_wino4_input_h2_dev(_p(x), B, H, W, Cin, _p(slot), _p(V2), s))
        _lib.check(lib.cslam_wino_zgemm_h2_dev(_p(V2), _p(U2[0]), T, Cin, Cout, _p(M), s))
        inv_su = U2[1]
    elif slot is not None:
        V3 = ws._buf("V", (36 * T * 3 * Cin + 1) // 2, x.device).view(torch.float16)[:36 * T * 3 * Cin].view(36, T, 3 * Cin)
        _lib.check(lib.cslam_wino4_input_h3_dev(_p(x), B, H, W, Cin, _p(slot), _p(V3), s))
        M = torch.bmm(V3, U3[0], out_dtype=torch.float32)
        inv_su = U3[1]
    else:
        n2, Uu, fin = (36, U4, lib.cslam_wino4_input_dev) if four else (16, U, lib.cslam_wino_input_dev)
        V = ws._buf("V", n2 * T * Cin, x.device).view(n2, T, Cin)
        M = ws._buf("M", n2 * T * Cout, x.device).view(n2, T, Cout)
        _lib.check(fin(_p(x), B, H, W, Cin, _p(V), s))
        torch.bmm(V, Uu, out=M)
    y = _out(B, Cout, H, W, pool, x.device)
    residual = _residual_like(residual, y)
    if z:
        _lib.check(lib.cslam_wino4_output_z_dev(_p(M), _po(bias), B, H, W, Cout, int(relu), int(pool), _p(slot), float(inv_su),
                                                _po(amax_out), _p(y), s))
    elif slot is not None or ws.amax_written:
        _lib.check(lib.cslam_wino4_output_scaled_dev(_p(M), _po(bias), _po(residual), B, H, W, Cout, int(relu), int(pool),
                                                     _po(slot), float(inv_su), _po(amax_out), _p(y), s))
    else:
        fout = lib.cslam_wino4_output_dev if four else lib.cslam_wino_output_dev
        _lib.check(fout(_p(M), _po(bias), _po(residual), B, H, W, Cout, int(relu), int(pool), _p(y), s))
    return y


class _Workspace(object):
    def __init__(self):
        self._ws = {}
        self.amax_written = False

    def _buf(self, name, numel, device):
        b = self._ws.get(name)
        if b is None or b.numel() < numel or b.device != device:
            b = torch.empty(numel, dtype=torch.float32, device=device)
            self._ws[name] = b
        return b[:numel]


def fold_bn(conv, bn):
    s = (bn.weight.double() / torch.sqrt(bn.running_var.double() + bn.eps))
    w = (conv.weight.double() * s[:, None, None, None]).float().contiguous(memory_format=torch.channels_last)
    b = bn.bias.double() - bn.running_mean.double() * s
    if conv.bias is not None:
        b = b + conv.bias.double() * s
    return w, b.float().contiguous()


class _FoldedConv(object):

    def __init__(self, conv, bn, tile, min_in_channels, direct=False):
        self.weight, self.bias = fold_bn(conv, bn)
        self.stride, self.padding = conv.stride, conv.padding
        self.U = self.U4 = self.Wg = self.Wp = None
        self.kernel = tuple(conv.kernel_size)
        self.wl1, self.bmax = out_bound(self.weight, self.bias)
        self.in_channels = conv.in_channels
        igemm_ok = (IGEMM_CONVS and conv.dilation == (1, 1) and conv.groups == 1 and conv.stride[0] == conv.stride[1]
                    and conv.padding[0] == conv.padding[1] and conv.out_channels % 64 == 0 and conv.weight.is_cuda
                    and (conv.in_channels % 32 == 0 or (conv.in_channels == 3 and 3 * conv.kernel_size[1] <= 32)))
        if direct and igemm_ok:
            self.Wg = igemm_pair_weights(self.weight)
            self.Wg = (self.Wg[0].to(self.weight.device), self.Wg[1])
            if (DIRECT_P and tuple(self.weight.shape) == (64, 64, 3, 3) and conv.stride == (1, 1) and conv.padding == (1, 1)):
                self.Wp = stem_direct_pair_weights(self.weight)
                self.Wp = (self.Wp[0].to(self.weight.device), self.Wp[1])
        elif (conv.kernel_size == (3, 3) and conv.stride == (1, 1) and conv.padding == (1, 1) and conv.dilation == (1, 1)
                and conv.groups == 1 and conv.in_channels >= min_in_channels and conv.in_channels % 4 == 0
                and conv.out_channels % 4 == 0 and conv.weight.is_cuda):
            self.U = wino_weights(self.weight).to(self.weight.device)
            self.U4 = wino_weights(self.weight, 4).to(self.weight.device) if tile == 4 else None
        elif igemm_ok:
            self.Wg = igemm_pair_weights(self.weight)
            self.Wg = (self.Wg[0].to(self.weight.device), self.Wg[1])

    def __call__(self, ws, x, relu, residual=None, amax_in=None, amax_out=None, pool=False):
        ws.amax_written = False
        if self.U is not None:
            return wino_conv3x3(ws, x.contiguous(memory_format=torch.channels_last), self.U, self.U4, self.bias, relu,
                                False, residual)
        if self.Wg is not None and x.shape[2] + 2 * self.padding[0] >= self.kernel[0] and x.shape[3] + 2 * self.padding[0] >= self.kernel[1]:
            y = conv_igemm(ws, x, self.Wg, self.bias, self.kernel, self.stride[0], self.padding[0], relu, residual, amax_in, amax_out, pool)
            ws.amax_written = amax_out is not None
            return y
        y = torch.nn.functional.conv2d(x, self.weight, self.bias, self.stride, self.padding)
        if residual is not None:
            y += residual
        return torch.relu_(y) if relu else y


class WinogradResNet(_Workspace):

    def __init__(self, trunk, min_in_channels=64, tile=4, direct=None):
        super().__init__()
        self.trunk, self.min_in_channels, self.tile = trunk, int(min_in_channels), int(tile)
        self.direct = IGEMM_CONVS if direct is None else bool(direct)
        use_tuned_gemms()
        self.refresh()

    def refresh(self):
        mods = list(self.trunk)
        mk = lambda c, b: _FoldedConv(c, b, self.tile, self.min_in_channels, self.direct)
        self.stem = mk(mods[0], mods[1])
        self.stem_pool = mods[3]
        self.blocks = []
        for layer in mods[4:]:
            for blk in layer:
                d = {"down": None if blk.downsample is None else mk(blk.downsample[0], blk.downsample[1]),
                     "c1": mk(blk.conv1, blk.bn1), "c2": mk(blk.conv2, blk.bn2),
                     "c3": mk(blk.conv3, blk.bn3) if hasattr(blk, "conv3") else None}
                self.blocks.append(d)
        return self

    @torch.no_grad()
    def __call__(self, x, x_bound=None):
        x = x.contiguous(memory_format=torch.channels_last)
        slots = self._buf("amax_slots", 4 * len(self.blocks) + 6, x.device)
        slots.zero_()
        free = iter(slots.split(1))

        def run(conv, inp, relu, res, a_in):
            out_slot = next(free)
            y = conv(self, inp, relu, res, a_in, out_slot)
            return y, (out_slot if self.amax_written else None)
        a0 = None
        if x_bound is not None:
            a0 = next(free)
            a0.fill_(float(x_bound))
        sp = self.stem_pool
        ho = (x.shape[2] + 2 * self.stem.padding[0] - self.stem.kernel[0]) // self.stem.stride[0] + 1
        wo = (x.shape[3] + 2 * self.stem.padding[1] - self.stem.kernel[1]) // self.stem.stride[1] + 1
        if (self.stem.Wg is not None and x.shape[1] == 3 and stem_pool_fits(ho, wo) and isinstance(sp, torch.nn.MaxPool2d)
                and _pair(sp.kernel_size) == (3, 3) and _pair(sp.stride) == (2, 2) and _pair(sp.padding) == (1, 1)
                and _pair(sp.dilation) == (1, 1) and not sp.ceil_mode):
            ax = next(free)
            x = self.stem(self, x, True, None, a0, ax, pool=True)
        else:
            y, ax = run(self.stem, x, True, None, a0)
            x = sp(y)
        convs = [c for b in self.blocks for c in (b["down"], b["c1"], b["c2"], b["c3"]) if c is not None]
        if PAIR_ACTS and ax is not None and all(c.Wg is not None and c.in_channels % 32 == 0 for c in convs):
            pslots = self._buf("pair_slots", 2 * len(convs) + 2, x.device)
            pslots.zero_()
            pfree = iter(pslots.split(1))
            last = convs[-1]

            def runp(conv, a, relu, res):
                amax_out, bound_out = next(pfree), next(pfree)
                if (conv.Wp is not None and (a.pairs or res is None) and conv is not last
                        and direct_p_fits(conv.weight.shape, conv.kernel, conv.stride[0], conv.padding[0], a.shape[2], a.shape[3])):
                    return conv3x3_direct_p(a, conv.Wp, conv.bias, relu, res, conv.wl1, conv.bmax, amax_out, bound_out, True)
                return conv_igemm_p(self, a, conv.Wg, conv.bias, conv.kernel, conv.stride[0], conv.padding[0], relu, res, conv.wl1,
                                    conv.bmax, amax_out, bound_out, conv is not last)
            cur = PairAct(x, False, x.shape, ax, ax)
            for b in self.blocks:
                idt = cur if b["down"] is None else runp(b["down"], cur, False, None)
                o = runp(b["c1"], cur, True, None)
                if b["c3"] is None:
                    cur = runp(b["c2"], o, True, idt)
                else:
                    o = runp(b["c2"], o, True, None)
                    cur = runp(b["c3"], o, True, idt)
            return cur.t
        for b in self.blocks:
            idt = x if b["down"] is None else run(b["down"], x, False, None, ax)[0]
            o, ao = run(b["c1"], x, True, None, ax)
            if b["c3"] is None:
                x, ax = run(b["c2"], o, True, idt, ao)
            else:
                o, ao = run(b["c2"], o, True, None, ao)
                x, ax = run(b["c3"], o, True, idt, ao)
        return x


class _Step(object):
    __slots__ = ("kind", "module", "conv", "relu", "pool", "U", "U4", "U3", "U2", "Up", "Uph", "bias", "stem", "Wd", "Wr", "Wdr", "Wdr2", "wl1", "bmax")

    def __init__(self):
        for name in self.__slots__:
            setattr(self, name, None)
        self.kind, self.relu, self.pool = "torch", False, False


def _wants(st):
    return st.U3 is not None or st.U2 is not None or st.Uph is not None or st.Wd is not None


TRUNK_FORMS = {"conv_direct": 1, "conv_direct_r": True, "conv_direct_r2": True, "stem_direct": True, "wino_stem": True, "fused_h": True, "split16_min_cin": None,
               "wino_chain": True}
CHAIN_TILE_COLS = (5, 16)
FP32_GEMM_FORMS = {"split16_min_cin": 0, "fused_h": False, "wino_stem": False}


def _pool2_at(mods, i):
    p = mods[i] if i < len(mods) else None
    return (isinstance(p, nn.MaxPool2d) and p.kernel_size in (2, (2, 2)) and p.stride in (2, (2, 2))
            and p.padding in (0, (0, 0)) and not p.ceil_mode)


class WinogradTrunk(_Workspace):

    def __init__(self, encoder, min_in_channels=256, tile=2, fused64=None, split16_h3=False, forms=None):
        super().__init__()
        self.encoder = encoder
        self.min_in_channels = int(min_in_channels)
        self.tile = int(tile)
        self.fused64 = True if fused64 is None else bool(fused64)
        self.fused_min_blocks = 256
        self.fused_couts = (64, 128)
        self.input_bound = None
        self.forms = dict(TRUNK_FORMS)
        self.forms.update(forms or {})
        assert set(self.forms) == set(TRUNK_FORMS), "unknown trunk form"
        self.direct128 = int(self.forms["conv_direct"]) != 0
        self.direct_cins = (128,) if int(self.forms["conv_direct"]) == 2 else (64, 128)
        self.split16_h3 = bool(split16_h3)
        self.split16_min_cin = (256 if self.split16_h3 else 128) if self.forms["split16_min_cin"] is None else int(self.forms["split16_min_cin"])
        use_tuned_gemms()
        self.refresh()

    def refresh(self):
        mods = list(self.encoder)
        self.steps = []
        i = 0
        while i < len(mods):
            m = mods[i]
            st = _Step()
            ok = (isinstance(m, nn.Conv2d) and m.kernel_size == (3, 3) and m.stride == (1, 1) and m.padding == (1, 1)
                  and m.dilation == (1, 1) and m.groups == 1 and m.in_channels >= self.min_in_channels
                  and m.in_channels % 4 == 0 and m.out_channels % 4 == 0 and m.weight.is_cuda)
            if ok:
                st.kind, st.conv, st.relu, st.pool = "wino", m, False, False
                st.U = wino_weights(m.weight).to(m.weight.device)
                st.U4 = wino_weights(m.weight, 4).to(m.weight.device) if self.tile == 4 else None
                if st.U4 is not None and 0 < self.split16_min_cin <= m.in_channels:
                    if not self.split16_h3 and m.in_channels % 32 == 0 and m.out_channels % 128 == 0:
                        st.U2 = split16_pair_weights(st.U4)
                    else:
                        st.U3 = split16_weights(st.U4)
                if self.fused64 and m.in_channels == 64 and m.out_channels in self.fused_couts:
                    t4 = self.tile == 4
                    st.Up = fused64_weights(st.U4 if t4 else st.U)
                    if t4 and self.forms["fused_h"]:
                        st.Uph = fused64_pair_weights(st.U4)
                if (self.direct128 and self.tile == 4 and m.out_channels == 128 and m.in_channels in self.direct_cins):
                    st.Wd = direct_pair_weights(m.weight)
                    if m.in_channels == 64 and self.forms["conv_direct_r"]:
                        st.Wdr = direct_r_pair_weights(m.weight)
                    if m.in_channels == 128 and self.forms["conv_direct_r2"]:
                        st.Wdr2 = direct_r2_pair_weights(m.weight)
                st.bias = None if m.bias is None else m.bias.detach().to(torch.float32).contiguous()
                st.wl1, st.bmax = out_bound(m.weight, m.bias)
                i += 1
                if i < len(mods) and isinstance(mods[i], nn.ReLU):
                    st.relu = True
                    i += 1
                    if _pool2_at(mods, i):
                        st.pool = True
                        i += 1
            elif (isinstance(m, nn.Conv2d) and m.in_channels == 3 and m.kernel_size == (3, 3) and m.stride == (1, 1)
                  and m.padding == (1, 1) and m.dilation == (1, 1) and m.groups == 1 and m.out_channels % 16 == 0
                  and m.out_channels <= 512 and m.weight.is_cuda and not (i + 2 < len(mods) and isinstance(
                      mods[i + 1], nn.ReLU) and isinstance(mods[i + 2], nn.MaxPool2d))):
                st.kind, st.conv = "c3", m
                st.U = m.weight.detach().to(torch.float32).permute(1, 2, 3, 0).reshape(27, m.out_channels).contiguous()
                st.bias = None if m.bias is None else m.bias.detach().to(torch.float32).contiguous()
                i += 1
                if i < len(mods) and isinstance(mods[i], nn.ReLU):
                    st.relu = True
                    i += 1
            elif (isinstance(m, nn.Conv2d) and m.groups == 1 and m.out_channels % 4 == 0 and m.bias is not None
                  and m.weight.is_cuda and i + 1 < len(mods) and isinstance(mods[i + 1], nn.ReLU)):
                st.kind, st.conv, st.relu = "direct", m, True
                st.bias = m.bias.detach().to(torch.float32).contiguous()
                i += 2
                if _pool2_at(mods, i):
                    st.pool = True
                    i += 1
            else:
                st.kind, st.module = "torch", m
                i += 1
            self.steps.append(st)
        if self.forms["wino_stem"]:
            for a, b in zip(self.steps, self.steps[1:]):
                if (a.kind == "c3" and a.relu and a.conv.out_channels == 64 and b.kind == "wino" and b.Uph is not None
                        and b.relu and b.conv.out_channels == 64):
                    a.stem = stem_pair_weights(a.conv.weight)
                    if self.forms["stem_direct"]:
                        a.Wr = stem_direct_pair_weights(b.conv.weight)
        return self

    def _chain_len(self, k, B, H, W):
        if not (self.forms["wino_chain"] and _f4_fits(B, H, W) and CHAIN_TILE_COLS[0] <= -(-W // 4) <= CHAIN_TILE_COLS[1]):
            return 1
        pair = lambda st_: (st_.kind == "wino" and st_.U2 is not None and st_.Wd is None and st_.Up is None
                            and not _z_form(st_.conv.in_channels, st_.conv.out_channels))
        n = 1
        while (k + n < len(self.steps) and pair(self.steps[k + n - 1]) and pair(self.steps[k + n])
               and self.steps[k + n - 1].relu and not self.steps[k + n - 1].pool):
            n += 1
        return n

    def _want(self, slots, j):
        return slots[j:j + 1] if j < len(self.steps) and _wants(self.steps[j]) else None


    def _stem_pair(self, k, x, slots):
        st, (B, _, H, W) = self.steps[k], x.shape
        nxt = self.steps[k + 1] if st.stem is not None else None
        if nxt is None or not (B * -(-H // 16) * -(-W // 16) >= self.fused_min_blocks and not (nxt.pool and (H % 2 or W % 2))
                               and B * H * W * 64 < 2 ** 31):
            return None
        slot = slots[k:k + 1]
        if self.input_bound is not None:
            slot.fill_(float(self.input_bound))
        else:
            _amax_slot(x, slot)
        want = self._want(slots, k + 2)
        if st.Wr is not None:
            y = conv_stem_direct_h(x, st.stem, st.bias, st.Wr, nxt.bias, nxt.pool, slot, want)
        else:
            y = wino_stem64_h(x, st.stem, st.bias, nxt.Uph, nxt.bias, nxt.pool, slot, want)
        return y, want is not None, 1

    def _first_layer(self, k, x, slots):
        st, (B, _, H, W) = self.steps[k], x.shape
        Cout = st.conv.out_channels
        y = _out(B, Cout, H, W, False, x.device)
        want = self._want(slots, k + 1) if Cout == 64 else None
        _lib.check(_lib.load().cslam_conv3x3_c3_amax_dev(_p(x), _p(st.U), _po(st.bias), B, H, W, Cout, int(st.relu), _p(y), _po(want),
                                                         _stream(x)))
        return y, want is not None, 0

    def _torch_direct(self, k, x):
        st = self.steps[k]
        c = st.conv
        x = torch.nn.functional.conv2d(x, c.weight, None, c.stride, c.padding, c.dilation)
        x = x.contiguous(memory_format=torch.channels_last)
        B, Cout, H, W = x.shape
        pool = st.pool and H % 2 == 0 and W % 2 == 0
        y = _out(B, Cout, H, W, True, x.device) if pool else x
        _lib.check(_lib.load().cslam_bias_act_pool_dev(_p(x), _p(st.bias), B, H, W, Cout, 1, int(pool), _p(y), _stream(x)))
        return (torch.nn.functional.max_pool2d(y, 2, 2) if st.pool and not pool else y), None, 0

    def _direct128(self, k, x, have, slots):
        st, (B, _, H, W) = self.steps[k], x.shape
        if not (st.Wd is not None and not (st.pool and (H % 2 or W % 2))
                and B * -(-H // 16) * -(-W // 16) >= self.fused_min_blocks and x.numel() % 4 == 0):
            return None
        slot = _amax_slot(x, slots[k:k + 1], have)
        nxt = self.steps[k + 1] if k + 1 < len(self.steps) else None
        if (VGG_PAIRS and st.Wdr is not None and st.relu and not st.pool and nxt is not None and nxt.Wd is not None
                and nxt.Wdr is None and nxt.conv.in_channels == 128 and H * W * 512 < 2 ** 31 - 16
                and not (nxt.pool and (H % 2 or W % 2))):
            bslot = self._buf("vgg_pair_bound", 1, x.device)
            xp = conv3x3_direct_r_pairs(x, st.Wdr, st.bias, st.wl1, st.bmax, slot, bslot)
            want = self._want(slots, k + 2)
            return conv3x3_direct_hp(xp, (B, 128, H, W), bslot, nxt.Wd, nxt.bias, nxt.relu, nxt.pool, want), want is not None, 1
        want = self._want(slots, k + 1)
        if st.Wdr is not None and H * W * 512 < 2 ** 31 - 16:
            y = conv3x3_direct_r(x, st.Wdr, st.bias, st.relu, st.pool, slot, want)
        elif st.Wdr2 is not None and H * W * 512 < 2 ** 31 - 16:
            y = conv3x3_direct_r2(x, st.Wdr2, st.bias, st.relu, st.pool, slot, want)
        else:
            y = conv3x3_direct_h(x, st.Wd, st.bias, st.relu, st.pool, slot, want)
        return y, want is not None, 0

    def _fused64(self, k, x, have, slots):
        st, (B, _, H, W) = self.steps[k], x.shape
        if st.Up is None or (st.pool and (H % 2 or W % 2)):
            return None
        bh, bw = (16, 16) if st.Up.shape[1] == 36 else (8, 16)
        if B * -(-H // bh) * -(-W // bw) * st.Up.shape[2] // 4 < self.fused_min_blocks:
            return None
        if st.Uph is None or x.numel() >= 2 ** 31:
            return wino_fused64(x, st.Up, st.bias, st.relu, st.pool), None, 0
        slot = _amax_slot(x, slots[k:k + 1], have)
        want = self._want(slots, k + 1)
        return wino_fused64_h(x, st.Uph, st.bias, st.relu, st.pool, slot, want), want is not None, 0

    def _winograd(self, k, x, have, slots):
        st = self.steps[k]
        n = self._chain_len(k, x.shape[0], x.shape[2], x.shape[3])
        if n == 1:
            want = self._want(slots, k + 1)
            y = wino_conv3x3(self, x, st.U, st.U4, st.bias, st.relu, st.pool, U3=st.U3, U2=st.U2,
                             amax_in=slots[k:k + 1] if have else None, amax_out=want)
            return y, want is not None and self.amax_written, 0
        _amax_slot(x, slots[k:k + 1], have)
        want = self._want(slots, k + n)
        chain = self.steps[k:k + n]
        y = _pair_pipeline(self, x, [(t.U2, t.bias, t.wl1, t.bmax) for t in chain], slots[k:k + n], chain[-1].relu, chain[-1].pool,
                           None, want)
        return y, want is not None, n - 1

    @torch.no_grad()
    def __call__(self, x):
        slots = have = None
        if any(_wants(st) for st in self.steps):
            slots = self._buf("amax_slots", len(self.steps) + 1, x.device)
            slots.zero_()
        k = 0
        while k < len(self.steps):
            st = self.steps[k]
            if st.kind == "c3":
                x = x.contiguous()
                x, have, ran = self._stem_pair(k, x, slots) or self._first_layer(k, x, slots)
            else:
                x = x.contiguous(memory_format=torch.channels_last)
                if st.kind == "torch":
                    x, have, ran = st.module(x), None, 0
                elif st.kind == "direct":
                    x, have, ran = self._torch_direct(k, x)
                else:
                    x, have, ran = (self._direct128(k, x, have, slots) or self._fused64(k, x, have, slots)
                                    or self._winograd(k, x, have, slots))
            k += 1 + ran
        return x
```

include/cslam_hip.h:

```cpp
#ifndef CSLAM_HIP_H
#define CSLAM_HIP_H

#include <stdint.h>

#ifdef __cplusplus
extern "C" {
#endif

#define CSLAM_OK 0
#define CSLAM_E_INVALID (-1)
#define CSLAM_E_HIP (-2)
#define CSLAM_E_NOMEM (-3)
#define CSLAM_E_DIM (-4)
#define CSLAM_E_UNSUPPORTED (-5)
#define CSLAM_E_GRAPH (-6)
#define CSLAM_E_LIMIT (-7)

#define CSLAM_F32 0
#define CSLAM_F64 1

#define CSLAM_MODE_AUTO 0
#define CSLAM_MODE_SCAN 1
#define CSLAM_MODE_MFMA 2

typedef struct cslam_bank cslam_bank_t;
typedef struct cslam_comm cslam_comm_t;

const char *cslam_last_error(void);
int cslam_version(void);
int cslam_device_count(int *count);
int cslam_device_info(int device, char *name, int name_len, int64_t *hbm_bytes, int *cu_count);

int cslam_bank_create(int device, int dim, int64_t capacity_hint, cslam_bank_t **out);
int cslam_bank_destroy(cslam_bank_t *bank);
int cslam_bank_size(const cslam_bank_t *bank, int64_t *n, int *dim);
int cslam_bank_clear(cslam_bank_t *bank);
int cslam_bank_add_host(cslam_bank_t *bank, const void *vecs, int dtype, int64_t n);
int cslam_bank_add_dev(cslam_bank_t *bank, const float *d_vecs, int64_t ld, int64_t n, void *stream);
int cslam_bank_read_host(const cslam_bank_t *bank, int64_t row0, int64_t nrows, float *out);
int cslam_bank_device_ptr(const cslam_bank_t *bank, const float **d_rows, int64_t *ld);

int cslam_bank_search_host(cslam_bank_t *bank, const void *queries, int q_dtype, int64_t nq,
                           int k, const int64_t *row_limit, int mode,
                           int64_t *out_idx, double *out_sim, int32_t *out_cnt);
int cslam_bank_search_dev(cslam_bank_t *bank, const void *d_queries, int q_dtype, int64_t ldq,
                          int64_t nq, int k, const int64_t *d_row_limit, int mode,
                          int64_t *d_out_idx, double *d_out_sim, int32_t *d_out_cnt,
                          void *stream);

int cslam_bank_search_multi_dev(cslam_bank_t *const *banks, int nb, const void *d_queries, int q_dtype, int64_t ldq,
                                int64_t nq, const int *k, const int64_t *const *d_row_limit, int mode,
                                int64_t *const *d_out_idx, double *const *d_out_sim, int32_t *const *d_out_cnt,
                                void *stream);
int cslam_bank_search_enqueue_dev(cslam_bank_t *bank, const void *d_queries, int q_dtype, int64_t ldq, int64_t nq, int k,
                                  const int64_t *d_row_limit, int mode, int64_t *d_out_idx, double *d_out_sim,
                                  int32_t *d_out_cnt, void *stream);
int cslam_bank_search_finish(cslam_bank_t *bank, int64_t *n_uncertified);
int cslam_bank_search_flag_copy_dev(cslam_bank_t *bank, int32_t *d_count, void *stream);
int cslam_bank_search_multi_enqueue_dev(cslam_bank_t *const *banks, int nb, const void *d_queries, int q_dtype, int64_t ldq,
                                        int64_t nq, const int *k, const int64_t *const *d_row_limit, int mode,
                                        int64_t *const *d_out_idx, double *const *d_out_sim, int32_t *const *d_out_cnt,
                                        void *stream);
int cslam_bank_search_multi_finish(cslam_bank_t *const *banks, int nb, int64_t *n_uncertified );
int cslam_bank_last_stats(cslam_bank_t *bank, int64_t stats[4]);
int cslam_bank_last_stage(cslam_bank_t *bank, int32_t info[4]);
int cslam_bank_last_kernel_ms(cslam_bank_t *bank, float *ms);
int cslam_topk_merge_dev(const int64_t *d_idx, const double *d_sim, const int32_t *d_cnt,
                         const int64_t *row_offset, int shards, int64_t nq, int k,
                         int64_t *d_out_idx, double *d_out_sim, int32_t *d_out_cnt, void *stream);

int cslam_l2_normalize_dev(float *d_x, int64_t n, int d, int64_t ld, float eps,
                           int zero_norm_to_one, void *stream);
int cslam_vlad_aggregate_dev(const float *d_feat, const float *d_assign_w, const float *d_assign_b,
                             const float *d_centroids, int B, int C, int P, int K,
                             float *d_out, int64_t ldo, void *stream);
int cslam_vlad_aggregate_nhwc_dev(const float *d_feat, const float *d_assign_w, const float *d_assign_b,
                                  const float *d_centroids, int B, int C, int P, int K,
                                  float *d_out, int64_t ldo, void *stream);
int cslam_gem_fc_head_dev(const float *d_feat, float p, float eps, const float *d_W,
                          const float *d_b, int B, int C, int P, int Dout,
                          float *d_out, void *stream);
int cslam_gem_fc_head_nhwc_dev(const float *d_feat, float p, float eps, const float *d_W,
                               const float *d_b, int B, int C, int P, int Dout,
                               float *d_out, void *stream);
int cslam_pca_project_dev(const float *d_x, int64_t ldx, const float *d_comp, int64_t ldc,
                          const float *d_mean_proj, const float *d_inv_scale, int B, int Din, int Dout,
                          float *d_out, void *stream);
int cslam_pca_project_pairs_dev(const float *d_x, int64_t ldx, float x_bound, const void *d_W2, float inv_sw, int S,
                                const float *d_mean_proj, const float *d_inv_scale, int B, int Din, int Dout,
                                float *d_out, void *stream);
int cslam_preprocess_dev(const uint8_t *d_img, int B, int H, int W, int crop, int out_hw,
                         const float mean[3], const float std_[3], float *d_out, void *stream);
int cslam_preprocess_nhwc_dev(const uint8_t *d_img, int B, int H, int W, int crop, int out_hw,
                              const float mean[3], const float std_[3], float *d_out, void *stream);

int cslam_mac_grad_dev(const double *d_fiedler, const int32_t *d_edge_i, const int32_t *d_edge_j,
                       const double *d_weights, int64_t m, double *d_grad, void *stream);
int cslam_csr_spmm_dev(const int64_t *d_indptr, const int32_t *d_indices, const double *d_data,
                       int64_t n, const double *d_x, int nvec, double *d_y, void *stream);

int cslam_csr_spmm4_dev(const int64_t *d_indptr, const int32_t *d_indices, const double *d_data,
                        int64_t n, const double *d_x, double *d_y, void *stream);

int cslam_block4_gram_dev(const double *d_A, const double *d_B, int64_t n, double *d_partial,
                          double *d_out20, void *stream);
int cslam_block4_affine_dev(const double *d_A, int64_t n, const double *d_M16, const double *d_shift4,
                            double *d_out, void *stream);
int cslam_block4_residual_dev(const double *d_W, const double *d_X, int64_t n, const double *d_y4,
                              double sigma, double *d_partial, double *d_out1, void *stream);

int cslam_block4_gram_sync(const double *d_A, const double *d_B, int64_t n, double *d_partial, double *d_out20,
                           double *h_out20, void *stream);
int cslam_block4_affine_host(const double *d_A, int64_t n, const double *h_M16, const double *h_shift4, double *d_out,
                             void *stream);
int cslam_block4_residual_sync(const double *d_W, const double *d_X, int64_t n, const double *h_y4, double sigma,
                               double *d_partial, double *d_out1, double *h_out1, void *stream);

int cslam_chain_forward_dev(const double *d_b, const uint8_t *d_is_junction, const double *d_r, int64_t n,
                            const int64_t *d_J, int nJ, const int *d_seg_start_of, const int *d_seg_end_of,
                            const int64_t *d_sa, const int64_t *d_sb, const double *d_Rl,
                            double *d_Bn, double *d_Qn, double *d_tmp, double *d_scratch, double *d_bt,
                            void *stream);
int cslam_chain_backward_dev(const double *d_xJ, const double *d_Bn, const double *d_Qn, const double *d_r,
                             const double *d_Rn, const int *d_jid, const int *d_seg_of, const int64_t *d_sa,
                             const int64_t *d_sb, const double *d_Rl, int64_t n, double *d_x, void *stream);
int cslam_chol_solve4_dev(const double *d_L, int64_t m, int64_t ld, int col_major, const double *d_dinv,
                          const double *d_dinvT, int bs, double *d_x, double *d_tmp, void *stream);

int cslam_fiedler(int64_t n, const int64_t *h_indptr, const int32_t *h_indices, const double *h_data, const double *h_x0,
                  uint32_t seed, double tol, int max_iters, double *h_lambda2, double *h_v, int *h_iters, void *stream);
int cslam_fiedler_start_block(uint32_t seed, int64_t n, double *h_x0);
int cslam_fiedler_release(void);

int cslam_mac_fw_subset(int64_t num_poses, int64_t n_fixed, const int64_t *fixed_i, const int64_t *fixed_j,
                        const double *fixed_w, int64_t n_cand, const int64_t *cand_i, const int64_t *cand_j,
                        const double *cand_w, const double *w_init, int64_t k, int max_iters, double duality_gap_tol,
                        double fiedler_tol, double *h_selected, double *h_w_unrounded, double *h_upper, int *h_iters,
                        void *stream);

int cslam_pgo_plan(int64_t n, int64_t nf, const int32_t *h_ei, const int32_t *h_ej, int64_t prior, int64_t *h_info);
int cslam_pgo_linearize_dev(const double *d_poses, const double *d_meas, const double *d_sigmas, const double *d_weights,
                            double *d_E, void *stream);
int cslam_pgo_system_host(double *h_Hdiag, double *h_g, double *h_Hoff, int32_t *h_pa, int32_t *h_pb, void *stream);
int cslam_pgo_solve_dev(double lambda, double *d_delta, int *h_status, double *h_predicted, void *stream);
int cslam_pgo_retract_dev(const double *d_poses, const double *d_delta, int64_t n, double *d_out, void *stream);
int cslam_pgo_cost_dev(const double *d_poses, const double *d_meas, const double *d_sigmas, const double *d_weights, double *d_E,
                       double *h_cost, void *stream);
int cslam_pgo_weights_dev(const double *d_E, int64_t nfac, double mu, double barc2, const uint8_t *d_known, double *d_w,
                          void *stream);
int cslam_pgo_optimize(int64_t n, int64_t nf, const int32_t *h_ei, const int32_t *h_ej, int64_t prior, double *h_poses,
                       const double *h_meas, const double *h_sigmas, const uint8_t *h_known, const double *h_params,
                       double *h_weights, double *h_info);
int cslam_pgo_trace(int32_t *h_out, int64_t cap, int64_t *h_count);
int cslam_pgo_release(void);

typedef struct cslam_scbank cslam_scbank_t;
int cslam_scbank_create(int device, int rings, int sectors, int64_t capacity_hint, cslam_scbank_t **out);
int cslam_scbank_destroy(cslam_scbank_t *bank);
int cslam_scbank_size(const cslam_scbank_t *bank, int64_t *n, int *rings, int *sectors);
int cslam_scbank_clear(cslam_scbank_t *bank);
int cslam_scbank_add_host(cslam_scbank_t *bank, const double *sc, int64_t n);
int cslam_scbank_add_dev(cslam_scbank_t *bank, const double *d_sc, int64_t n, void *stream);
int cslam_scbank_read_host(const cslam_scbank_t *bank, int64_t first, int64_t count, double *sc_out,
                           double *ringkeys_out);
int cslam_scbank_search_host(cslam_scbank_t *bank, const double *queries, int64_t nq, int num_candidates,
                             const int64_t *row_limit, int64_t *best_idx, double *best_sim,
                             int32_t *best_yaw, int64_t *cand, double *cdist, int32_t *cyaw);
int cslam_scbank_search_dev(cslam_scbank_t *bank, const double *d_queries, int64_t nq, int num_candidates,
                            const int64_t *d_row_limit, int64_t *d_best_idx, double *d_best_sim,
                            int32_t *d_best_yaw, int64_t *d_cand, double *d_cdist, int32_t *d_cyaw,
                            void *stream);

int cslam_scancontext_from_cloud_dev(const double *d_points, const int64_t *d_offsets, int n_frames,
                                     int rings, int sectors, double max_length, double *d_out,
                                     int32_t *d_status, void *stream);

int cslam_icp_correspondences_dev(const double *d_src, const int64_t *d_src_off, const double *d_dst,
                                  const int64_t *d_dst_off, int n_pairs, const double *d_T, double max_dist,
                                  int32_t *d_idx, double *d_dist2, void *stream);
int cslam_icp_register_dev(const double *d_src, const int64_t *d_src_off, const double *d_dst,
                           const int64_t *d_dst_off, int n_pairs, const double *d_init, const double *max_dist,
                           const int *max_iter, int n_stages, double rel_fitness, double rel_rmse, double *d_T_out,
                           double *d_stats_out, void *stream);
int cslam_icp_register_plane_dev(const double *d_src, const int64_t *d_src_off, const double *d_dst,
                                 const int64_t *d_dst_off, const double *d_dst_normals, int n_pairs,
                                 const double *d_init, const double *max_dist, const int *max_iter, int n_stages,
                                 double rel_fitness, double rel_rmse, double *d_T_out, double *d_stats_out, void *stream);

int cslam_voxel_downsample_dev(const double *d_points, const int64_t *d_offsets, int n_clouds, double voxel,
                               double *d_out, int64_t *d_out_offsets, int32_t *d_counts, int32_t *d_status,
                               const int64_t *h_offsets, void *stream);

int cslam_knn_radius_dev(const double *d_points, const int64_t *d_offsets, int n_clouds, double radius, int max_nn,
                         int32_t *d_idx, double *d_d2, int32_t *d_count, const int64_t *h_offsets, void *stream);
int cslam_normals_dev(const double *d_points, const int64_t *d_offsets, int n_clouds, const int32_t *d_idx,
                      const double *d_d2, const int32_t *d_count, int list_width, double radius, int max_nn,
                      const double *viewpoint, double *d_normals, const int64_t *h_offsets, void *stream);
int cslam_fpfh_dev(const double *d_points, const double *d_normals, const int64_t *d_offsets, int n_clouds,
                   const int32_t *d_idx, const double *d_d2, const int32_t *d_count, int list_width, double *d_fpfh,
                   double *d_spfh, const int64_t *h_offsets, void *stream);
int cslam_feature_match_dev(const double *d_a, const int64_t *d_a_off, const double *d_b, const int64_t *d_b_off,
                            int n_pairs, int dim, int32_t *d_nn01, int32_t *d_nn10, int32_t *d_pairs,
                            int32_t *d_pair_count, const int64_t *h_a_off, const int64_t *h_b_off, void *stream);

#define CSLAM_ROBUST_MAX_N 8192
#define CSLAM_ROBUST_DEFAULT_NODE_BUDGET 2097152
int cslam_robust_graph_dev(const double *d_ms, const double *d_md, const int64_t *d_off, const int32_t *d_count, int n_pairs,
                           double noise_bound, uint64_t *d_adj, int64_t *d_adj_off, int32_t *d_deg, const int64_t *h_off,
                           const int32_t *h_count, void *stream);
int cslam_robust_clique_dev(const uint64_t *d_adj, const int64_t *d_adj_off, const int32_t *d_deg, const int64_t *d_off,
                            const int32_t *d_count, int n_pairs, int64_t node_budget, int32_t *d_clique, int32_t *d_clique_size,
                            int32_t *d_certified, int64_t *d_nodes, const int64_t *h_off, const int32_t *h_count, void *stream);
int cslam_robust_rotation_dev(const double *d_ms, const double *d_md, const int64_t *d_off, const int32_t *d_clique,
                              const int32_t *d_clique_size, int n_pairs, double noise_bound, double *d_R, double *d_weights,
                              int32_t *d_iters, const int64_t *h_off, void *stream);
int cslam_robust_translation_dev(const double *d_ms, const double *d_md, const int64_t *d_off, const int32_t *d_clique,
                                 const int32_t *d_clique_size, const double *d_R, int n_pairs, double noise_bound, double *d_t,
                                 int32_t *d_set, const int64_t *h_off, void *stream);
int cslam_robust_fit_dev(const double *d_src, const int64_t *d_src_off, const double *d_dst, const int64_t *d_dst_off,
                         const int32_t *d_rows, const int64_t *d_row_off, const int32_t *d_count, int n_pairs, double noise_bound,
                         int64_t node_budget, double *d_T, int64_t *d_info, int32_t *d_clique, const int64_t *h_row_off,
                         const int32_t *h_count, void *stream);

int cslam_vis_match_dev(const uint8_t *d_desc_from, const int64_t *d_from_off, const uint8_t *d_desc_to, const int64_t *d_to_off,
                        int n_pairs, int desc_bytes, double nndr, int32_t *d_rows, int32_t *d_count, const int64_t *h_from_off,
                        const int64_t *h_to_off, void *stream);
int cslam_vis_pnp_dev(const double *d_points, const int64_t *d_points_off, const double *d_pixels, const int64_t *d_pixels_off,
                      const int32_t *d_rows, const int64_t *d_row_off, const int32_t *d_count, const double *d_cameras, int n_pairs,
                      int iterations, double reproj_error, int min_inliers, int refine_iterations, int refine_rounds, uint64_t seed,
                      double *d_T, int32_t *d_info, int32_t *d_flags, void *stream);
int cslam_vis_register_dev(const uint8_t *d_desc_from, const double *d_points_from, const int64_t *d_from_off,
                           const uint8_t *d_desc_to, const double *d_pixels_to, const int64_t *d_to_off, const double *d_cameras,
                           int n_pairs, int desc_bytes, double nndr, int iterations, double reproj_error, int min_inliers,
                           int refine_iterations, int refine_rounds, uint64_t seed, int32_t *d_rows, int32_t *d_count, double *d_T,
                           int32_t *d_info, int32_t *d_flags, const int64_t *h_from_off, const int64_t *h_to_off, void *stream);

int cslam_bias_act_pool_dev(const float *d_x, const float *d_bias, int B, int H, int W, int C, int relu,
                            int pool, float *d_y, void *stream);
int cslam_conv3x3_c3_dev(const float *d_x, const float *d_wt, const float *d_bias, int B, int H, int W,
                         int Cout, int relu, float *d_y, void *stream);
int cslam_wino_input_dev(const float *d_x, int B, int H, int W, int C, float *d_V, void *stream);
int cslam_wino_output_dev(const float *d_M, const float *d_bias, const float *d_residual, int B, int H, int W,
                          int C, int relu, int pool, float *d_y, void *stream);
int cslam_wino4_input_dev(const float *d_x, int B, int H, int W, int C, float *d_V, void *stream);
int cslam_wino4_output_dev(const float *d_M, const float *d_bias, const float *d_residual, int B, int H, int W,
                           int C, int relu, int pool, float *d_y, void *stream);
int cslam_absmax_dev(const float *d_x, int64_t n, unsigned *d_slot, void *stream);
int cslam_wino4_output_scaled_dev(const float *d_M, const float *d_bias, const float *d_residual, int B, int H, int W,
                                  int C, int relu, int pool, const unsigned *d_amax, float inv_su, unsigned *d_amax_out,
                                  float *d_y, void *stream);
int cslam_wino4_input_h2_dev(const float *d_x, int B, int H, int W, int C, const unsigned *d_amax, void *d_V2,
                             void *stream);
int cslam_wino_gemm_h2_dev(const void *d_V2, const void *d_U2, int64_t T, int Cin, int Cout, float *d_M, void *stream);
int cslam_wino4_chain_h2_dev(const float *d_M, const float *d_bias, int B, int H, int W, int C, const unsigned *d_vscale,
                             float inv_su, const unsigned *d_amax_x, float wl1, float bmax, unsigned *d_amax_out,
                             unsigned *d_bound_out, void *d_V2, void *stream);
int cslam_wino_zgemm_h2_dev(const void *d_V2, const void *d_U2, int64_t T, int Cin, int Cout, float *d_Z, void *stream);
int cslam_wino4_output_z_dev(const float *d_Z, const float *d_bias, int B, int H, int W, int C, int relu, int pool,
                             const unsigned *d_amax, float inv_su, unsigned *d_amax_out, float *d_y, void *stream);

int cslam_wino4_fused_c64_h_dev(const float *d_x, const void *d_Uh, const float *d_bias, const float *d_residual, int B,
                                int H, int W, int Cout, int relu, int pool, const unsigned *d_amax, float inv_su,
                                unsigned *d_amax_out, float *d_y, void *stream);
int cslam_conv3x3_direct_h_dev(const float *d_x, const void *d_w2, const float *d_bias, int B, int H, int W, int Cin, int Cout,
                               int relu, int pool, const unsigned *d_amax, float inv_sw, unsigned *d_amax_out, float *d_y,
                               void *stream);
int cslam_conv3x3_c3_amax_dev(const float *d_x, const float *d_wt, const float *d_bias, int B, int H, int W, int Cout,
                              int relu, float *d_y, unsigned *d_amax_out, void *stream);

int cslam_wino4_stem_c64_h_dev(const float *d_x0, const void *d_w1, const float *d_b1, const float *d_sumw, float inv_sw,
                               const void *d_Uh, const float *d_bias, int B, int H, int W, int pool,
                               const unsigned *d_amax_x0, float inv_su, unsigned *d_amax_out, float *d_y, void *stream);

int cslam_conv_igemm_h2_dev(const float *d_x, const void *d_w2, const float *d_bias, const float *d_res, int B, int H, int W,
                            int Cin, int Cout, int KH, int KW, int stride, int pad, int relu, const unsigned *d_amax_in,
                            float inv_sw, unsigned *d_amax_out, float *d_y, void *stream);
int cslam_conv_stem_pool_igemm_h2_dev(const float *d_x, const void *d_w2, const float *d_bias, int B, int H, int W, int Cout,
                                      int KH, int KW, int stride, int pad, const unsigned *d_amax_in, float inv_sw,
                                      unsigned *d_amax_out, float *d_y, void *stream);
int cslam_conv_igemm_h2p_dev(const void *d_x, int x_pairs, const unsigned *d_xbound, const void *d_w2, const float *d_bias,
                             const void *d_res, int res_pairs, const unsigned *d_res_bound, int B, int H, int W, int Cin,
                             int Cout, int KH, int KW, int stride, int pad, int relu, const unsigned *d_amax_in, float inv_sw,
                             float wl1, float bmax, unsigned *d_amax_out, int out_pairs, unsigned *d_bound_out, void *d_y,
                             void *stream);

int cslam_conv3x3_direct_r_dev(const float *d_x, const void *d_w2r, const float *d_bias, int B, int H, int W, int Cin, int Cout,
                               int relu, int pool, const unsigned *d_amax, float inv_sw, unsigned *d_amax_out, float *d_y,
                               void *stream);

int cslam_conv3x3_direct_r2_dev(const float *d_x, const void *d_w2r2, const float *d_bias, int B, int H, int W, int Cin, int Cout,
                                int relu, int pool, const unsigned *d_amax, float inv_sw, unsigned *d_amax_out, float *d_y,
                                void *stream);

int cslam_conv3x3_direct_r_pairs_dev(const float *d_x, const void *d_w2r, const float *d_bias, int B, int H, int W, int Cin, int Cout,
                                     const unsigned *d_amax, float inv_sw, float wl1, float bmax, unsigned *d_amax_out,
                                     unsigned *d_bound_out, void *d_y, void *stream);
int cslam_conv3x3_direct_hp_dev(const void *d_x, const unsigned *d_xbound, const void *d_w2, const float *d_bias, int B, int H, int W,
                                int Cin, int Cout, int relu, int pool, float inv_sw, unsigned *d_amax_out, float *d_y, void *stream);

int cslam_conv3x3_direct_p_dev(const void *d_x, int x_pairs, const unsigned *d_xbound, const void *d_w2r, const float *d_bias, const void *d_res,
                               int res_pairs, const unsigned *d_res_bound, int B, int H, int W, int Cin, int Cout, int relu,
                               const unsigned *d_amax_in, float inv_sw, float wl1, float bmax, unsigned *d_amax_out, int out_pairs,
                               unsigned *d_bound_out, void *d_y, void *stream);

int cslam_conv_stem_direct_h_dev(const float *d_x0, const void *d_w1, const float *d_b1, const float *d_sumw, float inv_sw1,
                                 const void *d_w2r, const float *d_bias, float inv_sw2, int B, int H, int W, int pool,
                                 const unsigned *d_amax_x0, unsigned *d_amax_out, float *d_y, void *stream);

int cslam_comm_unique_id(void *id128);
int cslam_comm_init(int world, int rank, const void *id128, int device, cslam_comm_t **out);
int cslam_comm_destroy(cslam_comm_t *comm);
int cslam_comm_info(const cslam_comm_t *comm, int *world, int *rank);
int cslam_allgather_queries_dev(cslam_comm_t *comm, const void *d_local, int64_t rows, int64_t row_bytes, void *d_all,
                                void *stream);
int cslam_exchange_lists_dev(cslam_comm_t *comm, const void *d_send, void *d_recv, int64_t bytes_per_rank, void *stream);

#ifdef __cplusplus
}
#endif
#endif
```

Measured before the change: 18570.

## Walk stem conv tiles in vertical strips and reuse first-layer halo rows

The fused stem kernel now gives each workgroup whole vertical strips of 8-row tiles instead of scattered tiles. Consecutive tiles in a strip copy the two overlapping first-layer rows from the previous patch buffer and skip recomputing those conv1 tiles (9 instead of 12 per tile). This cuts redundant first-layer MFMA work and input loads. The cost is coarser work units, which can hurt load balance when strips are few relative to CUs, plus a second code path selected at run time.

```diff
diff --git a/cslam_amd/_lib.py b/cslam_amd/_lib.py
--- a/cslam_amd/_lib.py
+++ b/cslam_amd/_lib.py
@@ -138,6 +138,7 @@
     "cslam_conv3x3_direct_r_dev": (_i, [_vp, _vp, _vp, _i, _i, _i, _i, _i, _i, _i, _vp, C.c_float, _vp, _vp, _vp]),
     "cslam_conv3x3_direct_r2_dev": (_i, [_vp, _vp, _vp, _i, _i, _i, _i, _i, _i, _i, _vp, C.c_float, _vp, _vp, _vp]),
     "cslam_conv_stem_direct_h_dev": (_i, [_vp, _vp, _vp, _vp, C.c_float, _vp, _vp, C.c_float, _i, _i, _i, _i, _vp, _vp, _vp, _vp]),
+    "cslam_conv_stem_direct_h_walk_dev": (_i, [_vp, _vp, _vp, _vp, C.c_float, _vp, _vp, C.c_float, _i, _i, _i, _i, _i, _vp, _vp, _vp, _vp]),
     "cslam_wino4_stem_c64_h_dev": (_i, [_vp, _vp, _vp, _vp, C.c_float, _vp, _vp, _i, _i, _i, _i, _vp, C.c_float, _vp, _vp, _vp]),
     "cslam_debug_wfh_prof_dev": (_i, [_vp]),
     "cslam_conv3x3_c3_amax_dev": (_i, [_vp, _vp, _vp, _i, _i, _i, _i, _i, _vp, _vp, _vp]),
diff --git a/cslam_amd/csrc/conv_direct_r.hip b/cslam_amd/csrc/conv_direct_r.hip
--- a/cslam_amd/csrc/conv_direct_r.hip
+++ b/cslam_amd/csrc/conv_direct_r.hip
@@ -501,7 +501,7 @@
     ARG_CHECK(Cin == 128 && Cout == 128, "Cin and Cout must be 128");
     ARG_CHECK(!pool || ((H % 2) == 0 && (W % 2) == 0), "pooling needs even H and W");
     ARG_CHECK(inv_sw > 0.0f, "inv_sw must be positive");
-    ARG_CHECK((int64_t)H * W * 512 < 0x7ffffff0ll, "one image's maps must stay below 2 GiB (32-bit buffer offsets)");
+    ARG_CHECK((int64_t)(H + 10) * W * 512 < 0x7ffffff0ll, "one image's maps must stay below 2 GiB (32-bit buffer offsets)");
     ConvDirectR2Args a;
     a.x = d_x; a.w2 = (const f16x8 *)d_w2r2; a.bias = d_bias; a.y = d_y;
     a.B = B; a.H = H; a.W = W;
@@ -553,7 +553,7 @@
     ARG_CHECK(Cin == 64 && Cout == 128, "Cin must be 64 and Cout 128");
     ARG_CHECK(!pool || ((H % 2) == 0 && (W % 2) == 0), "pooling needs even H and W");
     ARG_CHECK(inv_sw > 0.0f, "inv_sw must be positive");
-    ARG_CHECK((int64_t)H * W * 512 < 0x7ffffff0ll, "one image's maps must stay below 2 GiB (32-bit buffer offsets)");
+    ARG_CHECK((int64_t)(H + 10) * W * 512 < 0x7ffffff0ll, "one image's maps must stay below 2 GiB (32-bit buffer offsets)");
     ConvDirectRArgs a;
     a.x = d_x; a.w2 = (const f16x8 *)d_w2r; a.bias = d_bias; a.y = d_y;
     a.B = B; a.H = H; a.W = W;
diff --git a/cslam_amd/csrc/conv_stem_direct_h.hip b/cslam_amd/csrc/conv_stem_direct_h.hip
--- a/cslam_amd/csrc/conv_stem_direct_h.hip
+++ b/cslam_amd/csrc/conv_stem_direct_h.hip
@@ -18,11 +18,19 @@
 #define SD_IMGB (SD_IMG + SD_T9)
 #define SD_NPIX 180
 #define SD_LDS (2 * SD_PATCHB + 2 * SD_IMGB * 4)
+#define SD_HALO16 (2 * SD_RP / 16)
+
+__host__ __device__ constexpr int sd_tile(bool cont, int g, int i) {
+    return !cont ? 2 * g + i : g < 3 ? (i == 0 ? g : -1) : 2 * g - 3 + i;
+}
+static_assert(sd_tile(true, 5, 1) == 8 && sd_tile(false, 5, 1) == 11, "9 and 12 first-layer tiles");
+static_assert(SD_HALO16 > 512 && SD_HALO16 <= 768 && SD_HALO16 * 16 == 2 * SD_RP && 8 * SD_RP + SD_HALO16 * 16 == SD_PATCHB, "the halo copy reads rows 8 - 9 and writes rows 0 - 1 of a patch buffer");
+static_assert(16 * 8 + 15 == 8 * 18 - 1 && 2 * SD_RP + 7 * SD_RP + 17 * SD_PP + (7 << 4) + 8 + 128 + 8 <= SD_PATCHB, "the 9-tile writes stay in the buffer");
 
 struct StemDirectArgs {
     const float *x0; const unsigned *w1; const float *b1; const float *sumw; float inv_sw1;
     const f16x8 *w2; const float *bias; float inv_sw2;
-    int B, H, W, gxb, gyb, nblk;
+    int B, H, W, gxb, gyb, nstrip, reuse;
     const unsigned *amax_in; unsigned *amax_out; float *y;
 };
 
@@ -61,10 +69,10 @@
     const bool by_xcd = (gridDim.x & 7) == 0;
     const int wg_xcd = by_xcd ? (int)blockIdx.x & 7 : 0, wg_j = by_xcd ? (int)blockIdx.x >> 3 : (int)blockIdx.x;
     const int wg_per = by_xcd ? (int)gridDim.x >> 3 : (int)gridDim.x;
-    const int per_xcd = by_xcd ? (p.nblk + 7) >> 3 : p.nblk;
-    const int blk_beg = wg_xcd * per_xcd;
-    const int blk_cnt = min(per_xcd, p.nblk - blk_beg);
-    const int n_mine = blk_cnt > wg_j ? (blk_cnt - wg_j + wg_per - 1) / wg_per : 0;
+    const int per_xcd = by_xcd ? (p.nstrip + 7) >> 3 : p.nstrip;
+    const int strip_beg = wg_xcd * per_xcd;
+    const int strip_cnt = min(per_xcd, p.nstrip - strip_beg);
+    const int n_mine = strip_cnt > wg_j ? (strip_cnt - wg_j + wg_per - 1) / wg_per * p.gyb : 0;
     if (n_mine <= 0) return;
 
     f16x8 wr[9][2][2];
@@ -96,15 +104,17 @@
         e_dst[j] = e < SD_IMG ? (r * SD_IW + c) * 3 + ci : -1;
         e_rc[j] = (ci << 16) | (r << 8) | c;
     }
-    struct Blk { int img, by, bx; };
+    struct Blk { int img, by, bx; bool cont; };
     auto decode_blk = [&](int bi) {
-        int blk = wg_j + bi * wg_per;
-        blk = blk_beg + (blk < blk_cnt ? blk : blk_cnt - 1);
-        const int per_img = p.gxb * p.gyb;
+        const bool past = bi >= n_mine;
+        bi = past ? n_mine - 1 : bi;
+        const int s = bi / p.gyb;
+        const int strip = strip_beg + wg_j + s * wg_per;
         Blk b;
-        b.img = blk / per_img;
-        const int rem = blk - b.img * per_img;
-        b.by = rem / p.gxb; b.bx = rem - b.by * p.gxb;
+        b.by = bi - s * p.gyb;
+        b.img = strip / p.gxb;
+        b.bx = strip - b.img * p.gxb;
+        b.cont = (p.reuse != 0) & !past & (b.by != 0);
         return b;
     };
     float raw[3];
@@ -112,8 +122,8 @@
 #pragma unroll
         for (int j = 0; j < 3; ++j) {
             const int ci = e_rc[j] >> 16, r = (e_rc[j] >> 8) & 255, c = e_rc[j] & 255;
-            const int gy = b.by * 8 - 2 + r, gx = b.bx * 16 - 2 + c;
-            const bool in = (e_dst[j] >= 0) & (gy >= 0) & (gy < p.H) & (gx >= 0) & (gx < p.W);
+            const int gy = b.by * 8 - (b.cont ? 0 : 2) + r, gx = b.bx * 16 - 2 + c;
+            const bool in = (e_dst[j] >= 0) & (gy >= 0) & (gy < p.H) & (gx >= 0) & (gx < p.W) & !(b.cont & (r >= 10));
             raw[j] = in ? p.x0[((int64_t)(b.img * 3 + ci) * p.H + gy) * p.W + gx] : 0.0f;
         }
     };
@@ -139,18 +149,24 @@
     for (int i = tid; i < 2 * 20 * 5; i += 256)
         s_img_all[(i / 100) * SD_IMGB + SD_IMG + ((i % 100) / 5) * 17 + 12 + (i % 5)] = 0u;
     unsigned pk[2][8];
-    auto conv1_read = [&](int g, const unsigned *s_img) {
+    auto conv1_read = [&](auto cont_tag, int g, const unsigned *s_img) {
+        constexpr bool CONT = decltype(cont_tag)::value;
 #pragma unroll
         for (int i = 0; i < 2; ++i) {
-            const unsigned *ib = (const unsigned *)((const char *)s_img + c1_src[2 * g + i]);
+            const int t = sd_tile(CONT, g, i);
+            if (t < 0) continue;
+            const unsigned *ib = (const unsigned *)((const char *)s_img + c1_src[t]);
 #pragma unroll
             for (int j = 0; j < 8; ++j) pk[i][j] = ib[j];
         }
     };
     f32x4 c1[2];
     float c1v[2][4];
-    auto conv1_piece = [&](int g, int piece, const Blk &b, char *patch) {
+    auto conv1_piece = [&](auto cont_tag, int g, int piece, char *patch) {
+        constexpr bool CONT = decltype(cont_tag)::value;
         const int i = piece & 1;
+        const int t = sd_tile(CONT, g, i);
+        if (t < 0) return;
         if (piece < 2) {
             u32x4 ah, al;
 #pragma unroll
@@ -174,8 +190,8 @@
         const float d0 = sub_half<0>(c1v[i][0], h01), d1 = sub_half<1>(c1v[i][1], h01);
         const float d2 = sub_half<0>(c1v[i][2], h23), d3 = sub_half<1>(c1v[i][3], h23);
         const __half2 l01 = __floats2half2_rn(d0, d1), l23 = __floats2half2_rn(d2, d3);
-        if ((DBG & 16) == 0 && (2 * g + i < 11 || l15 < 4)) {
-            char *d = patch + c1_dst[2 * g + i];
+        if ((DBG & 16) == 0 && (t < 11 || l15 < 4)) {
+            char *d = patch + c1_dst[t];
             *(uint2 *)d = make_uint2(*(const unsigned *)&h01, *(const unsigned *)&h23);
             *(uint2 *)(d + 128) = make_uint2(*(const unsigned *)&l01, *(const unsigned *)&l23);
         }
@@ -251,13 +267,15 @@
         fh[SLOT] = *(const f16x8 *)(patch + fr_off[DX] + R * SD_RP + KS * 64);
         fl[SLOT] = *(const f16x8 *)(patch + fr_off[DX] + R * SD_RP + KS * 64 + 128);
     };
-    auto rstep = [&](auto col_tag, auto r_tag, const char *patch, const unsigned *s_img, const Blk &nblk, char *npatch) {
+    auto rstep = [&](auto cont_tag, auto col_tag, auto r_tag, const char *patch, const unsigned *s_img, char *npatch) {
         constexpr int COL = decltype(col_tag)::value, R = decltype(r_tag)::value;
+        constexpr bool CONT = decltype(cont_tag)::value;
         constexpr int DX = COL >> 1, KS = COL & 1, SLOT = (R + COL) % 3;
+        constexpr int NT = (sd_tile(CONT, COL, 0) >= 0) + (sd_tile(CONT, COL, 1) >= 0);
         if constexpr (DBG & 2) { }
         else if constexpr (R + 2 < 10) frag_read(col_tag, std::integral_constant<int, (R + 2) % 10>{}, patch);
         else if constexpr (COL < 5) frag_read(std::integral_constant<int, (COL + 1) % 6>{}, std::integral_constant<int, (R + 2) % 10>{}, patch);
-        if constexpr (R == 0 && !(DBG & 1) && !(DBG & 8)) conv1_read(COL, s_img);
+        if constexpr (R == 0 && !(DBG & 1) && !(DBG & 8)) conv1_read(cont_tag, COL, s_img);
 #pragma unroll
         for (int prod = 0; prod < 3; ++prod)
 #pragma unroll
@@ -268,10 +286,10 @@
                 const f16x8 b = prod == 1 ? fl[SLOT] : fh[SLOT];
                 acc[r] = __builtin_amdgcn_mfma_f32_16x16x32_f16(a, b, (COL == 0 && prod == 0 && dy == 0) ? (f32x4)(0.0f) : acc[r], 0, 0, 0);
             }
-        if constexpr (R >= 2 && R <= 7 && !(DBG & 1)) conv1_piece(COL, R - 2, nblk, npatch);
+        if constexpr (R >= 2 && R <= 7 && !(DBG & 1)) conv1_piece(cont_tag, COL, R - 2, npatch);
         if constexpr (COL < 2 && (R == 1 || R == 8)) epi_piece(2 * COL + (R == 8 ? 1 : 0));
-        __builtin_amdgcn_sched_group_barrier(0x100, R == 0 ? 18 : 2, 0);
-        constexpr int NM = 3 * ((R < 2 ? R + 1 : 3) - (R > 7 ? R - 7 : 0)) + ((R == 2 || R == 3) ? 3 : 0);
+        __builtin_amdgcn_sched_group_barrier(0x100, R == 0 ? 2 + 8 * NT : 2, 0);
+        constexpr int NM = 3 * ((R < 2 ? R + 1 : 3) - (R > 7 ? R - 7 : 0)) + (((R == 2 || R == 3) && sd_tile(CONT, COL, R - 2) >= 0) ? 3 : 0);
 #pragma unroll
         for (int m = 0; m < NM; ++m) {
             __builtin_amdgcn_sched_group_barrier(0x008, 1, 0);
@@ -280,12 +298,12 @@
         __builtin_amdgcn_sched_group_barrier(0x200, 2, 0);
         __builtin_amdgcn_sched_barrier(0);
     };
-    auto edge = [&](auto col_tag, const char *patch, const unsigned *s_img) {
+    auto edge = [&](auto cont_tag, auto col_tag, const char *patch, const unsigned *s_img) {
         constexpr int COL = decltype(col_tag)::value;
         constexpr int DX = COL >> 1, KS = COL & 1, SLOT = (9 + COL) % 3;
         constexpr int DX2 = (COL + 1) >> 1, KS2 = (COL + 1) & 1, SLOT2 = (COL + 1) % 3;
         if constexpr (!(DBG & 2)) frag_read(std::integral_constant<int, COL + 1>{}, std::integral_constant<int, 1>{}, patch);
-        if constexpr (!(DBG & 1) && !(DBG & 8)) conv1_read(COL + 1, s_img);
+        if constexpr (!(DBG & 1) && !(DBG & 8)) conv1_read(cont_tag, COL + 1, s_img);
 #pragma unroll
         for (int prod = 0; prod < 3; ++prod) {
             acc[7] = __builtin_amdgcn_mfma_f32_16x16x32_f16(prod == 2 ? wr[6 + DX][KS][1] : wr[6 + DX][KS][0], prod == 1 ? fl[SLOT] : fh[SLOT], acc[7], 0, 0, 0);
@@ -300,20 +318,43 @@
         }
         __builtin_amdgcn_sched_barrier(0);
     };
-    auto column = [&](auto col_tag, const char *patch, const unsigned *s_img, const Blk &nblk, char *npatch) {
+    auto column = [&](auto cont_tag, auto col_tag, const char *patch, const unsigned *s_img, char *npatch) {
         constexpr int COL_ = decltype(col_tag)::value;
-        if constexpr (COL_ == 0) rstep(col_tag, std::integral_constant<int, 0>{}, patch, s_img, nblk, npatch);
-        rstep(col_tag, std::integral_constant<int, 1>{}, patch, s_img, nblk, npatch);
-        rstep(col_tag, std::integral_constant<int, 2>{}, patch, s_img, nblk, npatch); rstep(col_tag, std::integral_constant<int, 3>{}, patch, s_img, nblk, npatch);
-        rstep(col_tag, std::integral_constant<int, 4>{}, patch, s_img, nblk, npatch); rstep(col_tag, std::integral_constant<int, 5>{}, patch, s_img, nblk, npatch);
-        rstep(col_tag, std::integral_constant<int, 6>{}, patch, s_img, nblk, npatch); rstep(col_tag, std::integral_constant<int, 7>{}, patch, s_img, nblk, npatch);
-        rstep(col_tag, std::integral_constant<int, 8>{}, patch, s_img, nblk, npatch);
-        if constexpr (COL_ == 5) rstep(col_tag, std::integral_constant<int, 9>{}, patch, s_img, nblk, npatch);
-        else edge(col_tag, patch, s_img);
+        if constexpr (COL_ == 0) rstep(cont_tag, col_tag, std::integral_constant<int, 0>{}, patch, s_img, npatch);
+        rstep(cont_tag, col_tag, std::integral_constant<int, 1>{}, patch, s_img, npatch);
+        rstep(cont_tag, col_tag, std::integral_constant<int, 2>{}, patch, s_img, npatch); rstep(cont_tag, col_tag, std::integral_constant<int, 3>{}, patch, s_img, npatch);
+        rstep(cont_tag, col_tag, std::integral_constant<int, 4>{}, patch, s_img, npatch); rstep(cont_tag, col_tag, std::integral_constant<int, 5>{}, patch, s_img, npatch);
+        rstep(cont_tag, col_tag, std::integral_constant<int, 6>{}, patch, s_img, npatch); rstep(cont_tag, col_tag, std::integral_constant<int, 7>{}, patch, s_img, npatch);
+        rstep(cont_tag, col_tag, std::integral_constant<int, 8>{}, patch, s_img, npatch);
+        if constexpr (COL_ == 5) rstep(cont_tag, col_tag, std::integral_constant<int, 9>{}, patch, s_img, npatch);
+        else edge(cont_tag, col_tag, patch, s_img);
     };
 #define SD_C(T) std::integral_constant<int, T>{}
-
-    [[maybe_unused]] unsigned long long t_main = 0, t_epi = 0, t_bar = 0, t1 = 0, t2 = 0, t3 = 0;
+    auto columns = [&](auto cont_tag, const char *patch, const unsigned *s_img, char *npatch) {
+        constexpr bool CONT = decltype(cont_tag)::value;
+        char *const c1patch = npatch + (CONT ? 2 * SD_RP : 0);
+        [[maybe_unused]] uint4 halo0, halo1, halo2;
+        [[maybe_unused]] const bool third = tid < SD_HALO16 - 512;
+        if constexpr (CONT) {
+            const char *src = patch + 8 * SD_RP + tid * 16;
+            halo0 = *(const uint4 *)src;
+            halo1 = *(const uint4 *)(src + 4096);
+            halo2 = *(const uint4 *)(src + (third ? 8192 : 0));
+        }
+        frag_read(SD_C(0), SD_C(0), patch);
+        frag_read(SD_C(0), SD_C(1), patch);
+        column(cont_tag, SD_C(0), patch, s_img, c1patch);
+        if constexpr (CONT) {
+            char *dst = npatch + tid * 16;
+            *(uint4 *)dst = halo0;
+            *(uint4 *)(dst + 4096) = halo1;
+            if (third) *(uint4 *)(dst + 8192) = halo2;
+            __builtin_amdgcn_sched_barrier(0);
+        }
+        column(cont_tag, SD_C(1), patch, s_img, c1patch); column(cont_tag, SD_C(2), patch, s_img, c1patch);
+        column(cont_tag, SD_C(3), patch, s_img, c1patch); column(cont_tag, SD_C(4), patch, s_img, c1patch); column(cont_tag, SD_C(5), patch, s_img, c1patch);
+    };
+    [[maybe_unused]] unsigned long long t_main = 0, t_epi = 0, t_bar = 0, t1 = 0, t2 = 0, t3 = 0, n_cont = 0;
     Blk cb = decode_blk(0);
     img_load(cb);
     img_store(s_img_all);
@@ -322,9 +363,9 @@
     __syncthreads();
 #pragma unroll
     for (int g = 0; g < 6; ++g) {
-        conv1_read(g, s_img_all);
-#pragma unroll
-        for (int piece = 0; piece < 6; ++piece) conv1_piece(g, piece, cb, sd_smem);
+        conv1_read(std::false_type{}, g, s_img_all);
+#pragma unroll
+        for (int piece = 0; piece < 6; ++piece) conv1_piece(std::false_type{}, g, piece, sd_smem);
         __builtin_amdgcn_sched_barrier(0);
     }
     border_fixup(cb, sd_smem);
@@ -338,10 +379,8 @@
         const Blk nnb = decode_blk(bi + 2);
         img_load(nnb);
         if (SD_PROF) t1 = __builtin_amdgcn_s_memtime();
-        frag_read(SD_C(0), SD_C(0), patch);
-        frag_read(SD_C(0), SD_C(1), patch);
-        column(SD_C(0), patch, s_img_next, nb, npatch); column(SD_C(1), patch, s_img_next, nb, npatch); column(SD_C(2), patch, s_img_next, nb, npatch);
-        column(SD_C(3), patch, s_img_next, nb, npatch); column(SD_C(4), patch, s_img_next, nb, npatch); column(SD_C(5), patch, s_img_next, nb, npatch);
+        if (nb.cont) columns(std::true_type{}, patch, s_img_next, npatch);
+        else columns(std::false_type{}, patch, s_img_next, npatch);
         if (!(DBG & 1)) border_fixup(nb, npatch);
         if (SD_PROF) { t2 = __builtin_amdgcn_s_memtime(); t_main += t2 - t1; }
         img_store(s_img_all + cur * SD_IMGB);
@@ -351,14 +390,14 @@
         e_ok = true;
         if (SD_PROF) { t3 = __builtin_amdgcn_s_memtime(); t_epi += t3 - t2; }
         __syncthreads();
-        if (SD_PROF) t_bar += __builtin_amdgcn_s_memtime() - t3;
+        if (SD_PROF) { t_bar += __builtin_amdgcn_s_memtime() - t3; n_cont += nb.cont; }
         cb = nb;
         nb = nnb;
     }
 #pragma unroll
     for (int k = 0; k < 4; ++k) epi_piece(k);
 #ifdef CSLAM_ABLATIONS
-    if (sd_prof && blockIdx.x == 0 && tid == 0) { sd_prof[0] = t_main; sd_prof[1] = t_epi; sd_prof[2] = t_bar; sd_prof[3] = 0; sd_prof[4] = (unsigned long long)n_mine; }
+    if (sd_prof && blockIdx.x == 0 && tid == 0) { sd_prof[0] = t_main; sd_prof[1] = t_epi; sd_prof[2] = t_bar; sd_prof[3] = n_cont; sd_prof[4] = (unsigned long long)n_mine; }
 #endif
 
     if (p.amax_out) {
@@ -374,9 +413,9 @@
     }
 }
 
-CSLAM_API int cslam_conv_stem_direct_h_dev(const float *d_x0, const void *d_w1, const float *d_b1, const float *d_sumw, float inv_sw1,
-                                           const void *d_w2r, const float *d_bias, float inv_sw2, int B, int H, int W, int pool,
-                                           const unsigned *d_amax_x0, unsigned *d_amax_out, float *d_y, void *stream) {
+static int stem_direct_launch(const float *d_x0, const void *d_w1, const float *d_b1, const float *d_sumw, float inv_sw1,
+                              const void *d_w2r, const float *d_bias, float inv_sw2, int B, int H, int W, int pool, int reuse_halo,
+                              const unsigned *d_amax_x0, unsigned *d_amax_out, float *d_y, void *stream) {
     PTR_DEVICE(d_x0);
     ARG_CHECK(d_x0 && d_w1 && d_sumw && d_w2r && d_y && d_amax_x0, "NULL argument");
     ARG_CHECK(B >= 1 && H >= 1 && W >= 1, "empty map");
@@ -388,13 +427,13 @@
     a.w2 = (const f16x8 *)d_w2r; a.bias = d_bias; a.inv_sw2 = inv_sw2;
     a.B = B; a.H = H; a.W = W;
     a.gxb = (int)ceil_div64(W, 16); a.gyb = (int)ceil_div64(H, 8);
-    const int64_t nblk = (int64_t)B * a.gxb * a.gyb;
-    ARG_CHECK(nblk < (1ll << 30), "too many blocks for one launch");
-    a.nblk = (int)nblk;
+    const int64_t nstrip = (int64_t)B * a.gxb;
+    ARG_CHECK(nstrip * a.gyb < (1ll << 30), "too many blocks for one launch");
+    a.nstrip = (int)nstrip; a.reuse = reuse_halo != 0;
     a.amax_in = d_amax_x0; a.amax_out = d_amax_out; a.y = d_y;
     const int n_cu = cslam_cu_count();
     ARG_CHECK(n_cu > 0, "no HIP device");
-    const int grid = (int)(nblk < n_cu ? nblk : n_cu);
+    const int grid = (int)(nstrip < n_cu ? nstrip : n_cu);
     hipStream_t st = (hipStream_t)stream;
     constexpr int lds = SD_LDS;
 #define SD_LAUNCH(P) do { \
@@ -425,3 +464,15 @@
     HIP_TRY(hipGetLastError());
     return CSLAM_OK;
 }
+
+CSLAM_API int cslam_conv_stem_direct_h_dev(const float *d_x0, const void *d_w1, const float *d_b1, const float *d_sumw, float inv_sw1,
+                                           const void *d_w2r, const float *d_bias, float inv_sw2, int B, int H, int W, int pool,
+                                           const unsigned *d_amax_x0, unsigned *d_amax_out, float *d_y, void *stream) {
+    return stem_direct_launch(d_x0, d_w1, d_b1, d_sumw, inv_sw1, d_w2r, d_bias, inv_sw2, B, H, W, pool, 1, d_amax_x0, d_amax_out, d_y, stream);
+}
+
+CSLAM_API int cslam_conv_stem_direct_h_walk_dev(const float *d_x0, const void *d_w1, const float *d_b1, const float *d_sumw, float inv_sw1,
+                                                const void *d_w2r, const float *d_bias, float inv_sw2, int B, int H, int W, int pool,
+                                                int reuse_halo, const unsigned *d_amax_x0, unsigned *d_amax_out, float *d_y, void *stream) {
+    return stem_direct_launch(d_x0, d_w1, d_b1, d_sumw, inv_sw1, d_w2r, d_bias, inv_sw2, B, H, W, pool, reuse_halo, d_amax_x0, d_amax_out, d_y, stream);
+}
diff --git a/cslam_amd/vpr/conv_kernels.py b/cslam_amd/vpr/conv_kernels.py
--- a/cslam_amd/vpr/conv_kernels.py
+++ b/cslam_amd/vpr/conv_kernels.py
@@ -156,13 +156,17 @@
     return y
 
 
-def conv_stem_direct_h(x0, stem, bias1, Wr, bias, pool, amax_x0, amax_out=None):
+def conv_stem_direct_h(x0, stem, bias1, Wr, bias, pool, amax_x0, amax_out=None, reuse_halo=True):
     B, C3, H, W = x0.shape
     assert C3 == 3 and x0.is_contiguous()
     y = _out(B, 64, H, W, pool, x0.device)
-    _lib.check(_lib.load().cslam_conv_stem_direct_h_dev(
-        _p(x0), _p(stem[0]), _po(bias1), _p(stem[2]), float(stem[1]), _p(Wr[0]), _po(bias), float(Wr[1]), B, H, W, int(pool),
-        _p(amax_x0), _po(amax_out), _p(y), _stream(x0)))
+    lib = _lib.load()
+    args = (_p(x0), _p(stem[0]), _po(bias1), _p(stem[2]), float(stem[1]), _p(Wr[0]), _po(bias), float(Wr[1]), B, H, W, int(pool))
+    tail = (_p(amax_x0), _po(amax_out), _p(y), _stream(x0))
+    if reuse_halo:
+        _lib.check(lib.cslam_conv_stem_direct_h_dev(*args, *tail))
+    else:
+        _lib.check(lib.cslam_conv_stem_direct_h_walk_dev(*args, 0, *tail))
     return y
 
 
diff --git a/cslam_amd/vpr/winograd.py b/cslam_amd/vpr/winograd.py
--- a/cslam_amd/vpr/winograd.py
+++ b/cslam_amd/vpr/winograd.py
@@ -286,8 +286,8 @@
     return st.U3 is not None or st.U2 is not None or st.Uph is not None or st.Wd is not None
 
 
-TRUNK_FORMS = {"conv_direct": 1, "conv_direct_r": True, "conv_direct_r2": True, "stem_direct": True, "wino_stem": True, "fused_h": True, "split16_min_cin": None,
-               "wino_chain": True}
+TRUNK_FORMS = {"conv_direct": 1, "conv_direct_r": True, "conv_direct_r2": True, "stem_direct": True, "stem_strips": True, "wino_stem": True, "fused_h": True,
+               "split16_min_cin": None, "wino_chain": True}
 CHAIN_TILE_COLS = (5, 16)
 FP32_GEMM_FORMS = {"split16_min_cin": 0, "fused_h": False, "wino_stem": False}
 
@@ -418,7 +418,7 @@
             _amax_slot(x, slot)
         want = self._want(slots, k + 2)
         if st.Wr is not None:
-            y = conv_stem_direct_h(x, st.stem, st.bias, st.Wr, nxt.bias, nxt.pool, slot, want)
+            y = conv_stem_direct_h(x, st.stem, st.bias, st.Wr, nxt.bias, nxt.pool, slot, want, bool(self.forms["stem_strips"]))
         else:
             y = wino_stem64_h(x, st.stem, st.bias, nxt.Uph, nxt.bias, nxt.pool, slot, want)
         return y, want is not None, 1
diff --git a/include/cslam_hip.h b/include/cslam_hip.h
--- a/include/cslam_hip.h
+++ b/include/cslam_hip.h
@@ -306,6 +306,9 @@
 int cslam_conv_stem_direct_h_dev(const float *d_x0, const void *d_w1, const float *d_b1, const float *d_sumw, float inv_sw1,
                                  const void *d_w2r, const float *d_bias, float inv_sw2, int B, int H, int W, int pool,
                                  const unsigned *d_amax_x0, unsigned *d_amax_out, float *d_y, void *stream);
+int cslam_conv_stem_direct_h_walk_dev(const float *d_x0, const void *d_w1, const float *d_b1, const float *d_sumw, float inv_sw1,
+                                      const void *d_w2r, const float *d_bias, float inv_sw2, int B, int H, int W, int pool,
+                                      int reuse_halo, const unsigned *d_amax_x0, unsigned *d_amax_out, float *d_y, void *stream);
 
 int cslam_comm_unique_id(void *id128);
 int cslam_comm_init(int world, int rank, const void *id128, int device, cslam_comm_t **out);
```

Result: no change. 18680, median of 6 (+0.6%).
